# marbl/Mash

Hardware: AMD Instinct MI355X
Metric: pairwise Mash distances/sec (s=1000) (higher is better)
Workload: dtype u64; 1 GPU; mash triangle all-vs-all, 100000 clustered synthetic sketches, k=21 s=1000, 4999950000 pairs/step, per-table job (index build + discover + fill + merge each step), row-block sharded x1; parallelism=rowblock1, rccl_ranks=0

## Files before the change

mash_amd/csrc/host_index.cpp:

```cpp
#include "host_internal.h"
#include "index_build.h"
#ifdef IX_PHASE_CLOCKS
namespace mg { void index_dump_clocks(); }
#endif
#include "sort_bits.h"

namespace {

const uint64_t kTilesLongestRun = 6144;
static const uint64_t kSplitMinRun = 128;

uint64_t longest_label_run(const uint32_t *lab_sorted, uint64_t n)
{
    if (!lab_sorted || n == 0) return 0;
    uint64_t run = 1, longest = 1;
    for (uint64_t a = 1; a < n; a++) {
        run = lab_sorted[a] == lab_sorted[a - 1] ? run + 1 : 1;
        longest = std::max(longest, run);
    }
    return longest;
}

struct SparseIndexBuild {
    mg_ctx *ctx;
    const mg_table *t;
    const uint32_t s;
    const bool clustered;
    const uint32_t split;
    mg_table::Sparse *sp;
    const uint64_t n;
    const std::chrono::steady_clock::time_point t_begin = std::chrono::steady_clock::now();
    bool stop = false;

    bool need_classes = false, dedup = true, want_dense = true, try_cluster = false, try_links = false;
    DevBuf<uint8_t> dc_cls, d_link;
    DevBuf<unsigned long long> dc_last, d_dig, d_dig_sorted, k_a, k_b;
    DevBuf<uint32_t> d_cnt, d_rows_sorted, d_flags, d_nflag, r_a, r_b, l_a, l_b, d_inv, d_lab;
    DevBuf<unsigned char> d_tmp_dup, d_tmp_cl;
    std::vector<uint8_t> hc_cls, link;
    std::vector<uint64_t> hc_last;
    std::vector<uint32_t> hc_nh, inv_v, lab_v;
    const uint32_t *inv = nullptr, *lab_sorted = nullptr;
    uint32_t nflag = 0;
    size_t tb_dup = 0, tb_cl = 0;
    bool cluster_q = false, links_q = false;

    const char *ix_mode = nullptr;
    bool ix_verify = false, ix_tiles = true;
    std::vector<uint32_t> cnt_true, cnt_perm;
    uint32_t max_cnt = 0;
    uint64_t maxv = 0, E_all = 0;
    double dens[65] = {0};
    double dens0 = 0;
    std::vector<uint32_t> rep;
    const uint64_t *H = nullptr;
    mg::IxPlan early_plan;
    DevBuf<unsigned char> d_lb;
    bool lb_made = false;
    bool cnt_stale = false;

    std::vector<uint32_t> cls_of, cls_off, cls_rows, cls_first;

    uint32_t E = 0, end_bit = 0, sort_begin_bit = 0;
    std::vector<mg::DenseGroup> cand_groups;
    std::vector<uint32_t> grp_of_h;
    DevBuf<mg::DenseGroup> d_groups;
    DevBuf<uint32_t> d_grp_of, d_lead_rows, d_val, d_valj, d_cnt_sub, d_off_sub, d_nlead;
    DevBuf<unsigned long long> d_key, d_keyj;
    uint32_t lead_lists = 0, lead_tot[2] = {0, 0}, lead_cap = 0;
    bool lead_ready = false, lead_done = false, cand_prepared = false;
    mg::IxPlan plan;
    size_t temp_bytes = 0;
    DevBuf<unsigned char> temp;
    DevBuf<uint32_t> gs_of;
    DevBuf<unsigned long long> key64_a, key64_b;
    struct Stat { unsigned long long shared; uint32_t max_group, groups, bad, tie_overflow; uint32_t ixf[4]; } h_stat = {0, 0, 0, 0, 0, {0, 0, 0, 0}};
    DevBuf<Stat> d_stat;
    DevBuf<unsigned char> d_slots;
    bool want_order = true, ok = false;
    size_t nshort = 0;
    std::vector<uint32_t> short_cnt;
    hipError_t e = hipSuccess;

    bool built = false;

    SparseIndexBuild(mg_ctx *c, const mg_table *tab, uint32_t sketch_size, bool clustered_variant, mg_table::Sparse *index, uint32_t split_row)
        : ctx(c), t(tab), s(sketch_size), clustered(clustered_variant), split(split_row), sp(index), n(tab->n), dc_cls(c), d_link(c), dc_last(c), d_dig(c),
          d_dig_sorted(c), k_a(c), k_b(c), d_cnt(c), d_rows_sorted(c), d_flags(c), d_nflag(c), r_a(c), r_b(c), l_a(c), l_b(c), d_inv(c),
          d_lab(c), d_tmp_dup(c), d_tmp_cl(c), d_lb(c), d_groups(c), d_grp_of(c), d_lead_rows(c), d_val(c), d_valj(c), d_cnt_sub(c),
          d_off_sub(c), d_nlead(c), d_key(c), d_keyj(c), temp(c), gs_of(c), key64_a(c), key64_b(c), d_stat(c), d_slots(c)
    {
    }

    int unusable(const char *why)
    {
        sp->usable = false;
        sp->why = why;
        stop = true;
        return MG_OK;
    }

    hipError_t counts_to_device()
    {
            if (!cnt_stale) return hipSuccess;
            cnt_stale = false;
            return hipMemcpyAsync(d_cnt, cnt_true.data(), n * 4, hipMemcpyHostToDevice, ctx->stream);
    }

    template <class T> bool take(T **p, size_t count)
    {
        void *q = nullptr;
        if (ctx_malloc(ctx, &q, std::max<size_t>(count, 1) * sizeof(T)) != hipSuccess) return false;
        *p = static_cast<T *>(q);
        return true;
    }

    void drop()
    {
            for (void **q : {(void **)&sp->off, (void **)&sp->keys_sorted, (void **)&sp->gend, (void **)&sp->sorted_rows, (void **)&sp->code_img,
                             (void **)&sp->pos_img, (void **)&sp->short_rows, (void **)&sp->short_cnt, (void **)&sp->counters, (void **)&sp->order,
                             (void **)&sp->rep, (void **)&sp->cls_of, (void **)&sp->cls_off, (void **)&sp->cls_rows, (void **)&sp->cls_first})
                if (*q) { ctx_free(ctx, *q); *q = nullptr; }
    }

    int scan_rows();
    int order_rows();
    int find_copies();
    int lay_out();
    void prepare_candidates();
    void finish_build();
    int build_by_tiles();
    int build_by_sort();
    int check_build();
    int dense_groups();
    int run();
};

int SparseIndexBuild::scan_rows()
{
    need_classes = t->cls.size() != n;
    dedup = !ctx_opt(ctx, "MASHGPU_SPARSE_NO_DEDUP");
    want_dense = true;
    if (const char *v = ctx_opt(ctx, "MASHGPU_COMPARE_DENSE")) want_dense = atoi(v) != 0;
    try_cluster = clustered && n >= 16;
    try_links = !try_cluster && want_dense && n >= 8 && s <= 16384;
    tb_dup = mg::sparse_dup_temp_bytes((uint32_t)n);
    tb_cl = mg::dense_cluster_temp_bytes((uint32_t)n);
    if (d_cnt.alloc(n) != hipSuccess || (need_classes && (dc_cls.alloc(n) != hipSuccess || dc_last.alloc(n) != hipSuccess)) ||
        (dedup && (d_dig.alloc(n) != hipSuccess || d_dig_sorted.alloc(n) != hipSuccess || d_rows_sorted.alloc(n) != hipSuccess ||
                   d_flags.alloc(n) != hipSuccess || d_nflag.alloc(1) != hipSuccess || d_tmp_dup.alloc(std::max<size_t>(tb_dup, 16)) != hipSuccess))) {
        (void)hipGetLastError();
        return unusable("no device memory for the index");
    }
    {
        hipError_t e = hipSuccess;
        if (need_classes) {
            hc_cls.resize(n);
            hc_last.resize(n);
            hc_nh.resize(n);
            e = mg::launch_row_classes(t->hashes, t->nhash, n, t->s, dc_cls, dc_last, ctx->stream);
        }
        if (e == hipSuccess) e = mg::launch_sparse_row_counts(t->nhash, (uint32_t)n, (uint32_t)std::min<uint64_t>(t->s, s), d_cnt, ctx->stream);
        if (e == hipSuccess && dedup) {
            e = mg::launch_sparse_row_digest(t->hashes, t->s, d_cnt, (uint32_t)n, d_dig, ctx->stream);
            if (e == hipSuccess)
                e = mg::launch_sparse_dup_suspects(d_dig, d_cnt, (uint32_t)n, d_tmp_dup, tb_dup, d_dig_sorted, d_rows_sorted, d_flags, d_nflag, ctx->stream);
        }
        if (e == hipSuccess && try_cluster) {
            if (k_a.alloc(4 * n) == hipSuccess && k_b.alloc(4 * n) == hipSuccess && r_a.alloc(4 * n) == hipSuccess && r_b.alloc(4 * n) == hipSuccess &&
                l_a.alloc(n) == hipSuccess && l_b.alloc(n) == hipSuccess && d_inv.alloc(n) == hipSuccess && d_lab.alloc(n) == hipSuccess &&
                d_tmp_cl.alloc(std::max<size_t>(tb_cl, 16)) == hipSuccess) {
                e = mg::dense_cluster_rows(t->hashes, t->s, d_cnt, (uint32_t)n, d_tmp_cl, tb_cl, k_a, k_b, r_a, r_b, l_a, l_b, d_inv, d_lab, ctx->stream, split);
                cluster_q = true;
            } else {
                (void)hipGetLastError();
            }
        }
        if (e == hipSuccess && try_links) {
            if (d_link.alloc(n) == hipSuccess) {
                link.resize(n);
                e = mg::launch_dense_neighbors(t->hashes, t->s, d_cnt, (uint32_t)n, d_link, ctx->stream);
                links_q = true;
            } else {
                (void)hipGetLastError();
            }
        }
        const size_t pin_bytes = 8 * n + 4 * n + 4 * n + 4 * n + 8 + n + n + 64;
        unsigned char *pin = static_cast<unsigned char *>(ctx_pinned(ctx, pin_bytes));
        unsigned long long *p_last = pin ? reinterpret_cast<unsigned long long *>(pin) : nullptr;
        uint32_t *p_nh = pin ? reinterpret_cast<uint32_t *>(pin + 8 * n) : nullptr, *p_inv = pin ? p_nh + n : nullptr, *p_lab = pin ? p_inv + n : nullptr;
        uint32_t *p_nflag = pin ? p_lab + n : &nflag;
        uint8_t *p_cls = pin ? pin + 20 * n + 8 : nullptr, *p_link = pin ? p_cls + n : nullptr;
        if (!pin) {
            if (cluster_q) { inv_v.resize(n); lab_v.resize(n); p_inv = inv_v.data(); p_lab = lab_v.data(); }
            p_nh = hc_nh.data(); p_cls = hc_cls.data(); p_last = reinterpret_cast<unsigned long long *>(hc_last.data()); p_link = link.data();
        }
        if (e == hipSuccess && need_classes) {
            e = hipMemcpyAsync(p_nh, t->nhash, n * 4, hipMemcpyDeviceToHost, ctx->stream);
            if (e == hipSuccess) e = hipMemcpyAsync(p_cls, dc_cls, n, hipMemcpyDeviceToHost, ctx->stream);
            if (e == hipSuccess) e = hipMemcpyAsync(p_last, dc_last, n * 8, hipMemcpyDeviceToHost, ctx->stream);
        }
        if (e == hipSuccess && dedup) e = hipMemcpyAsync(p_nflag, d_nflag, 4, hipMemcpyDeviceToHost, ctx->stream);
        if (e == hipSuccess && cluster_q) {
            e = hipMemcpyAsync(p_inv, d_inv, n * 4, hipMemcpyDeviceToHost, ctx->stream);
            if (e == hipSuccess) e = hipMemcpyAsync(p_lab, d_lab, n * 4, hipMemcpyDeviceToHost, ctx->stream);
        }
        if (e == hipSuccess && links_q) e = hipMemcpyAsync(p_link, d_link, n, hipMemcpyDeviceToHost, ctx->stream);
        const hipError_t es = hipStreamSynchronize(ctx->stream);
        if (e == hipSuccess) e = es;
        if (e == hipSuccess && pin) {
            if (need_classes) {
                memcpy(hc_nh.data(), p_nh, n * 4);
                memcpy(hc_cls.data(), p_cls, n);
                memcpy(hc_last.data(), p_last, n * 8);
            }
            if (dedup) nflag = *p_nflag;
            if (links_q) memcpy(link.data(), p_link, n);
        }
        if (cluster_q) { inv = p_inv; lab_sorted = p_lab; }
        if (e != hipSuccess) return fail(ctx, MG_ERR_HIP, std::string("compare (index: rows, copies, order): ") + hipGetErrorString(e));
    }
    if (need_classes) {
        t->cls.swap(hc_cls);
        t->last.swap(hc_last);
        t->nh.swap(hc_nh);
    }
    if (!links_q) link.clear();
    return MG_OK;
}

int SparseIndexBuild::order_rows()
{
    ix_mode = ctx_opt(ctx, "MASHGPU_SPARSE_INDEX");
    ix_verify = ix_mode && strcmp(ix_mode, "verify") == 0;
    ix_tiles = !ix_mode || strcmp(ix_mode, "sort") != 0;
    cnt_true.assign(n, 0);
    for (uint64_t i = 0; i < n; i++) {
        const uint32_t c = (uint32_t)std::min<uint64_t>(std::min<uint64_t>(t->nh[i], t->s), s);
        cnt_true[i] = c;
        E_all += c;
        max_cnt = std::max(max_cnt, c);
        if (c) {
            const uint64_t last = t->last[i];
            if (last == MG_HASH_PAD) return unusable("a hash equals the padding value");
            maxv = std::max(maxv, last);
            const double d = (double)c / ((double)last + 1.0);
            dens[64 - __builtin_clzll(last | 1ull)] += d;
            dens0 += d;
        }
    }
    H = t->hashes;
    bool keep_table_order = false;
    if (cluster_q && split != 0 && lab_sorted && !ctx_opt(ctx, "MASHGPU_SPLIT_ALWAYS") && longest_label_run(lab_sorted, n) * (uint64_t)s < kSplitMinRun * 1000ull) {
        keep_table_order = true;
        lab_sorted = nullptr;
    }
    if (cluster_q) {
        bool identity = true;
        for (uint64_t a = 0; a < n && identity; a++) identity = inv[a] == a;
        if (!identity && !keep_table_order) {
            void *pi = nullptr, *ph = nullptr;
            if (ctx_malloc(ctx, &pi, n * 4) != hipSuccess || ctx_malloc(ctx, &ph, std::max<uint64_t>(n * t->s, 1) * 8) != hipSuccess) {
                (void)hipGetLastError();
                ctx_free(ctx, pi);
                lab_sorted = nullptr;
            } else {
                sp->inv = static_cast<uint32_t *>(pi);
                sp->phashes = static_cast<uint64_t *>(ph);
                HIP_TRY(ctx, hipMemcpyAsync(sp->inv, d_inv, n * 4, hipMemcpyDeviceToDevice, ctx->stream));
                if (ix_tiles && !(dedup && nflag) && E_all > 0 && E_all < (1ull << 31) && longest_label_run(lab_sorted, n) <= kTilesLongestRun) {
                    early_plan = mg::index_plan((uint32_t)n, (uint32_t)E_all, s, sp->rs, t->s, maxv, dens0, ix_verify);
                    if (early_plan.ok && d_lb.alloc(early_plan.lb_bytes) == hipSuccess) {
                        HIP_TRY(ctx, mg::index_gather_rows(early_plan, t->hashes, sp->inv, d_cnt, sp->phashes, d_lb, ctx->stream));
                        lb_made = true;
                    } else {
                        (void)hipGetLastError();
                    }
                }
                if (!lb_made) HIP_TRY(ctx, mg::launch_dense_gather_rows(t->hashes, t->s, sp->inv, (uint32_t)n, sp->phashes, ctx->stream));
                H = sp->phashes;
                cnt_perm.resize(n);
                for (uint64_t a = 0; a < n; a++) cnt_perm[a] = cnt_true[inv[a]];
                cnt_true.swap(cnt_perm);
                cnt_stale = true;
            }
        }
    } else {
        lab_sorted = nullptr;
    }
    if (want_dense && n >= 8 && s <= 16384 && lab_sorted) {
        link.assign(n, 0);
        for (uint64_t a = 1; a < n; a++) link[a] = (a != split && lab_sorted[a] == lab_sorted[a - 1] && cnt_true[a] && cnt_true[a - 1]) ? 1 : 0;
    } else if (cluster_q && want_dense && n >= 8 && s <= 16384 && d_link.alloc(n) == hipSuccess) {
        link.resize(n);
        HIP_TRY(ctx, counts_to_device());
        HIP_TRY(ctx, mg::launch_dense_neighbors(H, t->s, d_cnt, (uint32_t)n, d_link, ctx->stream));
        HIP_TRY(ctx, hipMemcpyAsync(link.data(), d_link, n, hipMemcpyDeviceToHost, ctx->stream));
        HIP_TRY(ctx, hipStreamSynchronize(ctx->stream));
    } else if (!links_q) {
        (void)hipGetLastError();
        link.clear();
    }
    return MG_OK;
}

int SparseIndexBuild::find_copies()
{
    if (dedup && nflag) {
        HIP_TRY(ctx, counts_to_device());
        HIP_TRY(ctx, mg::launch_sparse_row_digest(H, t->s, d_cnt, (uint32_t)n, d_dig, ctx->stream));
        HIP_TRY(ctx, mg::launch_sparse_dup_suspects(d_dig, d_cnt, (uint32_t)n, d_tmp_dup, tb_dup, d_dig_sorted, d_rows_sorted, d_flags, d_nflag, ctx->stream));
        HIP_TRY(ctx, hipMemcpyAsync(&nflag, d_nflag, 4, hipMemcpyDeviceToHost, ctx->stream));
        HIP_TRY(ctx, hipStreamSynchronize(ctx->stream));
        if (nflag) {
            std::vector<uint32_t> rows_sorted(n), flags(n);
            HIP_TRY(ctx, hipMemcpyAsync(rows_sorted.data(), d_rows_sorted, n * 4, hipMemcpyDeviceToHost, ctx->stream));
            HIP_TRY(ctx, hipMemcpyAsync(flags.data(), d_flags, n * 4, hipMemcpyDeviceToHost, ctx->stream));
            HIP_TRY(ctx, hipStreamSynchronize(ctx->stream));
            std::vector<uint2> pairs;
            pairs.reserve(nflag);
            for (uint64_t k = 1, g0 = 0; k < n; k++) {
                if (flags[k]) pairs.push_back(make_uint2(rows_sorted[k], rows_sorted[g0]));
                else g0 = k;
            }
            DevBuf<uint2> d_pairs(ctx);
            DevBuf<uint32_t> d_eq(ctx);
            if (d_pairs.alloc(pairs.size()) != hipSuccess || d_eq.alloc(pairs.size()) != hipSuccess) { (void)hipGetLastError(); return unusable("no device memory for the index"); }
            std::vector<uint32_t> eq(pairs.size());
            HIP_TRY(ctx, hipMemcpyAsync(d_pairs, pairs.data(), pairs.size() * sizeof(uint2), hipMemcpyHostToDevice, ctx->stream));
            HIP_TRY(ctx, mg::launch_sparse_row_equal(H, t->s, d_cnt, d_pairs, (uint32_t)pairs.size(), d_eq, ctx->stream));
            HIP_TRY(ctx, hipMemcpyAsync(eq.data(), d_eq, pairs.size() * 4, hipMemcpyDeviceToHost, ctx->stream));
            HIP_TRY(ctx, hipStreamSynchronize(ctx->stream));
            for (size_t k = 0; k < pairs.size(); k++)
                if (eq[k]) {
                    if (rep.empty()) { rep.resize(n); for (uint64_t i = 0; i < n; i++) rep[i] = (uint32_t)i; }
                    rep[pairs[k].x] = pairs[k].y;
                    sp->copies++;
                }
        }
    }
    if (sp->copies) {
        cls_of.assign(n, 0xFFFFFFFFu);
        std::vector<uint32_t> size(n, 0);
        for (uint64_t i = 0; i < n; i++) size[rep[i]]++;
        uint32_t ncls = 0, tot = 0;
        for (uint64_t i = 0; i < n; i++)
            if (size[i] >= 2) { cls_of[i] = ncls++; cls_off.push_back(tot); tot += size[i]; }
        cls_off.push_back(tot);
        cls_rows.resize(tot);
        std::vector<uint32_t> fillp(cls_off.begin(), cls_off.end() - 1);
        for (uint64_t i = 0; i < n; i++) {
            const uint32_t k = cls_of[rep[i]];
            if (k != 0xFFFFFFFFu) cls_rows[fillp[k]++] = (uint32_t)i;
        }
        cls_first.resize(tot);
        for (uint32_t k = 0; k < ncls; k++) {
            const uint64_t m = cls_off[k + 1] - cls_off[k];
            sp->cls_pairs += m * (m - 1) / 2;
            for (uint32_t u = cls_off[k]; u < cls_off[k + 1]; u++) cls_first[u] = cls_off[k];
        }
        sp->cls_members = tot;
        if (ncls == 1 && tot == n && cnt_true[0] > 0) sp->one_class = (uint32_t)cnt_true[0];
        if (sp->one_class && ctx->aside_all_copies) ctx->aside_all_copies(sp->one_class);
    }
    return MG_OK;
}

int SparseIndexBuild::lay_out()
{
    uint64_t E64 = 0;
    sp->off_host.resize(n + 1);
    for (uint64_t i = 0; i < n; i++) {
        sp->off_host[i] = (uint32_t)E64;
        const uint64_t c = cnt_true[i];
        if (rep.empty() || rep[i] == i) E64 += c;
        if (E64 >= (1ull << 31)) return unusable("2^31 entries or more");
        if (c < s) sp->short_rows_host.push_back((uint32_t)i);
        if (c == 0) sp->has_empty = true;
    }
    sp->off_host[n] = (uint32_t)E64;
    if (E64 == 0) return unusable("no hashes");
    E = (uint32_t)E64;
    sp->E = E;
    end_bit = (uint32_t)(64 - __builtin_clzll(maxv | 1ull));
    sort_begin_bit = mg::sparse_sort_begin_bit(E, end_bit, ctx_opt(ctx, "MASHGPU_SPARSE_SORT_BITS"), ctx_opt(ctx, "MASHGPU_SPARSE_SORT_ALL_BITS") != nullptr);
    if (sort_begin_bit > 0 && !ctx_opt(ctx, "MASHGPU_SPARSE_SORT_BITS")) sort_begin_bit = mg::sort_begin_bit_from_density(dens, end_bit, sort_begin_bit);
    lead_lists = mg::dense_sublists();
    lead_cap = std::max<uint32_t>(E / 4u / lead_lists + 64u, 256u);
    if (const char *ev = ctx_opt(ctx, "MASHGPU_DENSE_LEAD_CAP")) lead_cap = std::max<uint32_t>((uint32_t)atoi(ev), 1u);
    const bool tiles_hopeless = ix_tiles && !ix_verify && lab_sorted && !ctx_opt(ctx, "MASHGPU_SPARSE_INDEX") &&
                                longest_label_run(lab_sorted, n) > kTilesLongestRun;
    if (ix_tiles && !tiles_hopeless) plan = mg::index_plan((uint32_t)n, E, s, sp->rs, t->s, maxv, dens0, ix_verify);
    else if (tiles_hopeless) plan.why = "a clade of more rows than a bucket's sort takes";
    if (lb_made && !(plan.ok && memcmp(&plan.g, &early_plan.g, sizeof plan.g) == 0)) lb_made = false;
    temp_bytes = std::max(std::max(mg::sparse_order_temp_bytes((uint32_t)n), mg::sparse_order_slice_temp_bytes((uint32_t)n)),
                          mg::sparse_offsets_temp_bytes((uint32_t)n));
    want_order = !ctx_opt(ctx, "MASHGPU_SPARSE_NO_ORDER");
    ok = temp.alloc(std::max<size_t>(temp_bytes, 16)) == hipSuccess && gs_of.alloc(E) == hipSuccess && d_stat.alloc(1) == hipSuccess &&
              d_slots.alloc(std::max(mg::sparse_stat_scratch_bytes(), mg::index_stat_scratch_bytes())) == hipSuccess &&
              (!want_order || (key64_a.alloc(n) == hipSuccess && key64_b.alloc(n) == hipSuccess));
    ok = ok && take(&sp->off, n + 1) && take(&sp->keys_sorted, E) && take(&sp->gend, E) && take(&sp->sorted_rows, E) &&
         take(&sp->code_img, (size_t)n * sp->rs + 64) && take(&sp->pos_img, (size_t)n * sp->rs) && take(&sp->counters, 4) &&
         (!want_order || take(&sp->order, n));
    nshort = sp->short_rows_host.size();
    short_cnt.assign(nshort, 0);
    for (size_t k = 0; k < nshort; k++) short_cnt[k] = cnt_true[sp->short_rows_host[k]];
    if (ok && nshort) ok = take(&sp->short_rows, nshort) && take(&sp->short_cnt, nshort);
    if (ok && sp->copies)
        ok = take(&sp->rep, n) && take(&sp->cls_of, n) && take(&sp->cls_off, cls_off.size()) && take(&sp->cls_rows, cls_rows.size()) &&
             take(&sp->cls_first, cls_first.size());
    e = hipSuccess;
    if (ok && sp->copies) {
        e = hipMemcpyAsync(sp->rep, rep.data(), n * 4, hipMemcpyHostToDevice, ctx->stream);
        if (e == hipSuccess) e = hipMemcpyAsync(sp->cls_of, cls_of.data(), n * 4, hipMemcpyHostToDevice, ctx->stream);
        if (e == hipSuccess) e = hipMemcpyAsync(sp->cls_off, cls_off.data(), cls_off.size() * 4, hipMemcpyHostToDevice, ctx->stream);
        if (e == hipSuccess) e = hipMemcpyAsync(sp->cls_rows, cls_rows.data(), cls_rows.size() * 4, hipMemcpyHostToDevice, ctx->stream);
        if (e == hipSuccess) e = hipMemcpyAsync(sp->cls_first, cls_first.data(), cls_first.size() * 4, hipMemcpyHostToDevice, ctx->stream);
    }
    if (ok && e == hipSuccess) {
        if (rep.empty()) e = mg::launch_sparse_offsets(d_cnt, cnt_stale ? sp->inv : nullptr, (uint32_t)n, temp, sp->off, ctx->stream);
        else e = hipMemcpyAsync(sp->off, sp->off_host.data(), (n + 1) * 4, hipMemcpyHostToDevice, ctx->stream);
        if (e == hipSuccess && nshort) e = hipMemcpyAsync(sp->short_rows, sp->short_rows_host.data(), nshort * 4, hipMemcpyHostToDevice, ctx->stream);
        if (e == hipSuccess && nshort) e = hipMemcpyAsync(sp->short_cnt, short_cnt.data(), nshort * 4, hipMemcpyHostToDevice, ctx->stream);
    }
    return MG_OK;
}

void SparseIndexBuild::prepare_candidates()
{
    if (cand_prepared) return;
    cand_prepared = true;
    if (link.empty() || sp->copies != 0) return;
    for (uint64_t i = 1; i < n;) {
        if (!link[i]) { i++; continue; }
        uint64_t j = i;
        while (j < n && link[j]) j++;
        if (j - (i - 1) >= 8) {
            mg::DenseGroup g{};
            g.g0 = (uint32_t)(i - 1); g.g1 = (uint32_t)j;
            cand_groups.push_back(g);
        }
        i = j + 1;
    }
    if (cand_groups.empty()) return;
    const uint32_t ng = (uint32_t)cand_groups.size();
    grp_of_h.assign(n, 0xFFFFFFFFu);
    for (uint32_t g = 0; g < ng; g++)
        for (uint32_t r = cand_groups[g].g0; r < cand_groups[g].g1; r++) grp_of_h[r] = g;
    const uint64_t room = (uint64_t)lead_lists * lead_cap;
    if (d_groups.alloc(ng) == hipSuccess && d_grp_of.alloc(n) == hipSuccess && d_lead_rows.alloc(4 * n) == hipSuccess && d_nlead.alloc(2) == hipSuccess && d_cnt_sub.alloc(lead_lists) == hipSuccess &&
        d_off_sub.alloc(lead_lists) == hipSuccess && d_key.alloc(room) == hipSuccess && d_val.alloc(room) == hipSuccess && d_keyj.alloc(room) == hipSuccess &&
        d_valj.alloc(room) == hipSuccess &&
        hipMemcpyAsync(d_groups, cand_groups.data(), ng * sizeof(mg::DenseGroup), hipMemcpyHostToDevice, ctx->stream) == hipSuccess &&
        mg::launch_dense_group_rows(d_groups, ng, (uint32_t)n, d_grp_of, d_lead_rows, ctx->stream) == hipSuccess &&
        hipMemsetAsync(d_cnt_sub, 0, lead_lists * 4, ctx->stream) == hipSuccess && hipMemsetAsync(d_nlead, 0, 8, ctx->stream) == hipSuccess) {
        lead_ready = true;
    } else {
        (void)hipGetLastError();
        cand_groups.clear();
    }
}

void SparseIndexBuild::finish_build()
{
    if (e == hipSuccess && want_order)
        e = mg::launch_sparse_row_order(sp->off, sp->code_img, sp->gend, sp->rep, (uint32_t)n, sp->rs, temp, temp_bytes, key64_a, key64_b,
                                        sp->order, ctx->stream);
    if (e == hipSuccess) e = hipMemcpyAsync(&h_stat, d_stat, sizeof(Stat), hipMemcpyDeviceToHost, ctx->stream);
    if (e == hipSuccess) e = hipStreamSynchronize(ctx->stream);
}

int SparseIndexBuild::build_by_tiles()
{
    if (ok && e == hipSuccess && plan.ok) {
        DevBuf<unsigned char> d_tcnt(ctx), d_start(ctx), d_big(ctx), d_pk(ctx), d_tc(ctx);
        if ((lb_made || d_lb.alloc(plan.lb_bytes) == hipSuccess) && d_tcnt.alloc(plan.cnt_bytes) == hipSuccess && d_start.alloc(plan.start_bytes) == hipSuccess &&
            d_big.alloc(plan.big_bytes) == hipSuccess && d_pk.alloc(plan.pk_bytes) == hipSuccess && d_tc.alloc(plan.tc_bytes) == hipSuccess) {
            e = hipMemsetAsync(d_stat, 0, sizeof(Stat), ctx->stream);
            if (e == hipSuccess)
                e = mg::index_build(plan, H, sp->off, d_lb, d_tcnt, d_start, d_big, d_pk, d_tc, sp->keys_sorted, sp->sorted_rows, sp->gend, gs_of, sp->code_img,
                                    sp->pos_img, d_slots, &d_stat.p->shared, &d_stat.p->max_group, &d_stat.p->groups, d_stat.p->ixf, nullptr, ctx->stream,
                                    lb_made ? 1 | 8 : 1);
            DevBuf<uint32_t> d_swapped(ctx);
            if (e == hipSuccess && ctx_opt(ctx, "MASHGPU_IX_DEBUG_SWAP") && d_swapped.alloc(1) == hipSuccess) {
                e = hipMemsetAsync(d_swapped, 0, 4, ctx->stream);
                if (e == hipSuccess) e = mg::index_debug_swap(plan, d_pk, d_start, d_swapped, ctx->stream);
            }
            prepare_candidates();
            mg::IxLeaders lead;
            if (lead_ready) {
                lead.grp_of = d_lead_rows;
                lead.key = d_key;
                lead.val = d_val;
                lead.cnt = d_cnt_sub;
                lead.cap_sub = lead_cap;
                lead.nsub = lead_lists;
            }
            if (e == hipSuccess && ctx->aside_at_sort) ctx->aside_at_sort();
            if (e == hipSuccess)
                e = mg::index_build(plan, H, sp->off, d_lb, d_tcnt, d_start, d_big, d_pk, d_tc, sp->keys_sorted, sp->sorted_rows, sp->gend, gs_of, sp->code_img,
                                    sp->pos_img, d_slots, &d_stat.p->shared, &d_stat.p->max_group, &d_stat.p->groups, d_stat.p->ixf,
                                    lead_ready ? &lead : nullptr, ctx->stream, 2);
            if (e == hipSuccess && lead_ready) {
                e = mg::dense_join_leaders(d_key, d_val, lead_cap, d_keyj, d_valj, d_cnt_sub, d_off_sub, d_nlead, ctx->stream);
                if (e == hipSuccess) e = hipMemcpyAsync(lead_tot, d_nlead, 8, hipMemcpyDeviceToHost, ctx->stream);
            }
            hipEvent_t ev_stats = nullptr;
            if (e == hipSuccess) e = hipMemcpyAsync(&h_stat, d_stat, sizeof(Stat), hipMemcpyDeviceToHost, ctx->stream);
            if (e == hipSuccess) e = hipEventCreateWithFlags(&ev_stats, hipEventDisableTiming);
            if (e == hipSuccess) e = hipEventRecord(ev_stats, ctx->stream);
            if (e == hipSuccess)
                e = mg::index_build(plan, H, sp->off, d_lb, d_tcnt, d_start, d_big, d_pk, d_tc, sp->keys_sorted, sp->sorted_rows, sp->gend, gs_of, sp->code_img,
                                    sp->pos_img, d_slots, &d_stat.p->shared, &d_stat.p->max_group, &d_stat.p->groups, d_stat.p->ixf,
                                    lead_ready ? &lead : nullptr, ctx->stream, 4);
            if (e == hipSuccess && want_order)
                e = mg::launch_sparse_row_order(sp->off, sp->code_img, sp->gend, sp->rep, (uint32_t)n, sp->rs, temp, temp_bytes, key64_a, key64_b,
                                                sp->order, ctx->stream);
            if (ev_stats) {
                const hipError_t ew = e == hipSuccess ? hipEventSynchronize(ev_stats) : hipStreamSynchronize(ctx->stream);
                if (e == hipSuccess) e = ew;
                (void)hipEventDestroy(ev_stats);
            } else {
                (void)hipStreamSynchronize(ctx->stream);
            }
            built = e == hipSuccess && !h_stat.ixf[mg::IXF_DEGENERATE];
            if (built && lead_ready && lead_tot[1] > lead_cap && h_stat.ixf[mg::IXF_NBIG] == 0) {
                e = hipStreamSynchronize(ctx->stream);
                const uint32_t want_cap = lead_tot[1];
                for (void **q : {(void **)&d_key.p, (void **)&d_val.p, (void **)&d_keyj.p, (void **)&d_valj.p})
                    if (*q) { ctx_free(ctx, *q); *q = nullptr; }
                const uint64_t room = (uint64_t)lead_lists * want_cap;
                if (e == hipSuccess && d_key.alloc(room) == hipSuccess && d_val.alloc(room) == hipSuccess && d_keyj.alloc(room) == hipSuccess &&
                    d_valj.alloc(room) == hipSuccess) {
                    lead_cap = want_cap;
                    lead.key = d_key;
                    lead.val = d_val;
                    lead.cap_sub = lead_cap;
                    e = hipMemsetAsync(d_cnt_sub, 0, lead_lists * 4, ctx->stream);
                    if (e == hipSuccess) e = hipMemsetAsync(d_nlead, 0, 8, ctx->stream);
                    if (e == hipSuccess) e = hipMemsetAsync(d_stat.p, 0, offsetof(Stat, bad), ctx->stream);
                    if (e == hipSuccess)
                        e = mg::index_build(plan, H, sp->off, d_lb, d_tcnt, d_start, d_big, d_pk, d_tc, sp->keys_sorted, sp->sorted_rows, sp->gend, gs_of,
                                            sp->code_img, sp->pos_img, d_slots, &d_stat.p->shared, &d_stat.p->max_group, &d_stat.p->groups, d_stat.p->ixf, &lead,
                                            ctx->stream, 2);
                    if (e == hipSuccess) e = mg::dense_join_leaders(d_key, d_val, lead_cap, d_keyj, d_valj, d_cnt_sub, d_off_sub, d_nlead, ctx->stream);
                    if (e == hipSuccess) e = hipMemcpyAsync(lead_tot, d_nlead, 8, hipMemcpyDeviceToHost, ctx->stream);
                    if (e == hipSuccess) e = hipMemcpyAsync(&h_stat, d_stat, sizeof(Stat), hipMemcpyDeviceToHost, ctx->stream);
                    if (e == hipSuccess) e = hipStreamSynchronize(ctx->stream);
                    built = e == hipSuccess && !h_stat.ixf[mg::IXF_DEGENERATE];
                    if (ctx_opt(ctx, "MASHGPU_SPARSE_DBG"))
                        fprintf(stderr, "compare dense: a list of leaders asked for %u entries: found again with that room (%u leaders)\n", want_cap, lead_tot[0]);
                } else {
                    (void)hipGetLastError();
                }
            }
            lead_done = built && lead_ready;
            if (ctx_opt(ctx, "MASHGPU_SPARSE_DBG"))
                fprintf(stderr, "compare sparse: index by tiles: shift %u, %u buckets (%u per window, %u windows), fullest %u, %u beyond the LDS (%u values streamed)%s\n",
                        plan.g.shift, plan.g.Bp, plan.g.BW, plan.g.NW, h_stat.ixf[mg::IXF_MAXBUCKET], h_stat.ixf[mg::IXF_NBIG], h_stat.ixf[mg::IXF_NSTREAMED],
                        h_stat.ixf[mg::IXF_DEGENERATE] ? " -- clumped values: sorted instead" : "");
        } else {
            (void)hipGetLastError();
        }
    } else if (ix_tiles && ctx_opt(ctx, "MASHGPU_SPARSE_DBG")) {
        fprintf(stderr, "compare sparse: index by tiles refused: %s\n", plan.why);
    }
    sp->by_tiles = built;
    prepare_candidates();
#ifdef IX_PHASE_CLOCKS
    if (built && ctx_opt(ctx, "MASHGPU_IX_CLOCKS")) mg::index_dump_clocks();
#endif
    if (ix_verify && !built && ok && e == hipSuccess && !ctx_opt(ctx, "MASHGPU_SPARSE_INDEX_MAY_REFUSE"))
        return fail(ctx, MG_ERR_INVALID, std::string("index verify: the tile build refused this table (") + (plan.ok ? "bucket flags" : plan.why) + ")");
    return MG_OK;
}

int SparseIndexBuild::build_by_sort()
{
    if (ok && e == hipSuccess && (!built || ix_verify)) {
        const size_t sort_bytes = mg::sparse_sort_temp_bytes(E, end_bit, sort_begin_bit);
        DevBuf<unsigned char> temp_sort(ctx), d_ties(ctx);
        DevBuf<uint64_t> keys_a(ctx), v_keys(ctx);
        DevBuf<uint32_t> idx_a(ctx), idx_sorted(ctx), v_rows(ctx), v_gend(ctx), v_gs(ctx), v_code(ctx), v_pos(ctx);
        DevBuf<unsigned long long> d_diff(ctx);
        bool ok2 = temp_sort.alloc(std::max<size_t>(sort_bytes, 16)) == hipSuccess && keys_a.alloc(E) == hipSuccess && idx_a.alloc(E) == hipSuccess &&
                   idx_sorted.alloc(E) == hipSuccess && d_ties.alloc(mg::sparse_tie_scratch_bytes()) == hipSuccess;
        if (ok2 && built)
            ok2 = v_keys.alloc(E) == hipSuccess && v_rows.alloc(E) == hipSuccess && v_gend.alloc(E) == hipSuccess && v_gs.alloc(E) == hipSuccess &&
                  v_code.alloc((size_t)n * sp->rs + 64) == hipSuccess && v_pos.alloc((size_t)n * sp->rs) == hipSuccess && d_diff.alloc(16) == hipSuccess;
        if (!ok2) {
            (void)hipGetLastError();
            ok = false;
        } else {
            const Stat tiles_stat = h_stat;
            uint64_t *o_keys = built ? v_keys.p : sp->keys_sorted;
            uint32_t *o_rows = built ? v_rows.p : sp->sorted_rows, *o_gend = built ? v_gend.p : sp->gend, *o_gs = built ? v_gs.p : gs_of.p,
                     *o_code = built ? v_code.p : sp->code_img, *o_pos = built ? v_pos.p : sp->pos_img;
            for (uint32_t begin_bit = sort_begin_bit;; begin_bit = 0) {
                if (e == hipSuccess) e = hipMemsetAsync(d_stat, 0, sizeof(Stat), ctx->stream);
                if (e == hipSuccess)
                    e = mg::sparse_build_index(H, t->s, sp->off, (uint32_t)n, E, sp->rs, end_bit, temp_sort, sort_bytes, keys_a, idx_a, o_keys, idx_sorted,
                                               idx_a, o_gs, o_rows, o_gend, o_code, o_pos, d_slots, begin_bit, d_ties, &d_stat.p->shared,
                                               &d_stat.p->max_group, &d_stat.p->groups, &d_stat.p->bad, &d_stat.p->tie_overflow, ctx->stream);
                if (built) {
                    if (e == hipSuccess) e = hipMemcpyAsync(&h_stat, d_stat, sizeof(Stat), hipMemcpyDeviceToHost, ctx->stream);
                    if (e == hipSuccess) e = hipStreamSynchronize(ctx->stream);
                } else {
                    finish_build();
                }
                if (e != hipSuccess || (!h_stat.tie_overflow && !h_stat.bad) || begin_bit == 0) break;
                if (ctx_opt(ctx, "MASHGPU_SPARSE_DBG"))
                    fprintf(stderr, "compare sparse: sort on bits [%u, %u) %s: every bit again\n", begin_bit, end_bit,
                            h_stat.bad ? "left values out of order" : "left ties the repair could not take");
            }
            if (built && e == hipSuccess) {
                unsigned long long diff[16];
                for (int k = 0; k < 8; k++) { diff[2 * k] = 0; diff[2 * k + 1] = ~0ull; }
                e = hipMemcpyAsync(d_diff, diff, sizeof diff, hipMemcpyHostToDevice, ctx->stream);
                const uint64_t img = (uint64_t)n * sp->rs;
                if (e == hipSuccess) e = mg::index_verify_words((const uint32_t *)sp->keys_sorted, (const uint32_t *)v_keys.p, nullptr, 0, 2ull * E, d_diff.p + 0, ctx->stream);
                if (e == hipSuccess) e = mg::index_verify_words(sp->sorted_rows, v_rows, nullptr, 0, E, d_diff.p + 2, ctx->stream);
                if (e == hipSuccess) e = mg::index_verify_words(gs_of, v_gs, nullptr, 0, E, d_diff.p + 4, ctx->stream);
                if (e == hipSuccess) e = mg::index_verify_words(sp->gend, v_gend, v_gs, 1, E, d_diff.p + 6, ctx->stream);
                if (e == hipSuccess) e = mg::index_verify_words(sp->code_img, v_code, nullptr, 0, img, d_diff.p + 8, ctx->stream);
                if (e == hipSuccess) e = mg::index_verify_words(sp->pos_img, v_pos, v_code, 2, img, d_diff.p + 10, ctx->stream);
                if (e == hipSuccess) e = hipMemcpyAsync(diff, d_diff, sizeof diff, hipMemcpyDeviceToHost, ctx->stream);
                if (e == hipSuccess) e = hipStreamSynchronize(ctx->stream);
                if (e == hipSuccess) {
                    static const char *names[6] = {"values (32-bit words)", "rows", "group starts", "group ends", "code image", "position image"};
                    std::string msg;
                    for (int k = 0; k < 6; k++)
                        if (diff[2 * k]) msg += std::string(msg.empty() ? "" : "; ") + names[k] + ": " + std::to_string(diff[2 * k]) + " differ, first at " + std::to_string(diff[2 * k + 1]);
                    if (h_stat.shared != tiles_stat.shared || h_stat.max_group != tiles_stat.max_group || h_stat.groups != tiles_stat.groups)
                        msg += std::string(msg.empty() ? "" : "; ") + "statistics: shared " + std::to_string(tiles_stat.shared) + " / " + std::to_string(h_stat.shared) +
                               ", largest group " + std::to_string(tiles_stat.max_group) + " / " + std::to_string(h_stat.max_group) + ", groups " +
                               std::to_string(tiles_stat.groups) + " / " + std::to_string(h_stat.groups);
                    if (!msg.empty()) {
                        char geom[160];
                        snprintf(geom, sizeof geom, " [n %llu, E %u, shift %u, %u buckets, %u per window, %u windows]", (unsigned long long)n, E, plan.g.shift, plan.g.Bp, plan.g.BW, plan.g.NW);
                        sp->usable = false;
                        return fail(ctx, MG_ERR_INVALID, "index verify: tiles / sort -- " + msg + geom);
                    }
                }
            }
        }
    }
    return MG_OK;
}

int SparseIndexBuild::check_build()
{
    if (!ok) { (void)hipGetLastError(); drop(); return unusable("no device memory for the index"); }
    if (e != hipSuccess) { drop(); return fail(ctx, MG_ERR_HIP, std::string("compare (index build): ") + hipGetErrorString(e)); }
    if (h_stat.bad) { drop(); return unusable("sort order inside a value not by row"); }
    sp->G = h_stat.groups;
    sp->shared = h_stat.shared;
    sp->max_group = h_stat.max_group;
    sp->build_ms = std::chrono::duration<double, std::milli>(std::chrono::steady_clock::now() - t_begin).count();
    sp->usable = true;
    return MG_OK;
}

int SparseIndexBuild::dense_groups()
{
    if (!cand_groups.empty()) {
        auto t_dense = std::chrono::steady_clock::now();
        while (!cand_groups.empty()) {
            const uint32_t ng = (uint32_t)cand_groups.size();
            std::vector<uint32_t> &grp_of = grp_of_h;
            DevBuf<uint32_t> d_us(ctx), d_ue(ctx);
            DevBuf<unsigned long long> d_key2(ctx);
            DevBuf<unsigned char> d_tmp(ctx);
            if (d_us.alloc(ng) != hipSuccess || d_ue.alloc(ng) != hipSuccess) { (void)hipGetLastError(); break; }
            const uint32_t L = lead_lists;
            uint32_t *tot = lead_tot, cap_sub = lead_cap;
            hipError_t e2 = hipSuccess;
            if (!lead_done) {
                if (built || !lead_ready) break;
                for (int attempt = 0; e2 == hipSuccess; attempt++) {
                    if (attempt > 0) {
                        for (void **q : {(void **)&d_key.p, (void **)&d_val.p, (void **)&d_keyj.p, (void **)&d_valj.p})
                            if (*q) { ctx_free(ctx, *q); *q = nullptr; }
                        const uint64_t room = (uint64_t)L * cap_sub;
                        if (d_key.alloc(room) != hipSuccess || d_val.alloc(room) != hipSuccess || d_keyj.alloc(room) != hipSuccess || d_valj.alloc(room) != hipSuccess) {
                            (void)hipGetLastError();
                            e2 = hipErrorOutOfMemory;
                            break;
                        }
                    }
                    e2 = mg::dense_find_leaders(sp->sorted_rows, gs_of, sp->gend, d_grp_of, d_groups, E, d_key, d_val, cap_sub, d_keyj, d_valj, d_cnt_sub, d_off_sub,
                                                d_nlead, ctx->stream);
                    if (e2 == hipSuccess) e2 = hipMemcpyAsync(tot, d_nlead, 8, hipMemcpyDeviceToHost, ctx->stream);
                    if (e2 == hipSuccess) e2 = hipStreamSynchronize(ctx->stream);
                    if (e2 != hipSuccess || tot[1] <= cap_sub || attempt >= 1) break;
                    cap_sub = tot[1];
                }
            } else if (tot[1] > cap_sub && ctx_opt(ctx, "MASHGPU_SPARSE_DBG")) {
                fprintf(stderr, "compare dense: a list of leaders asked for %u entries, room for %u: no dense groups for this table\n", tot[1], cap_sub);
            }
            const uint32_t nlead = tot[0];
            if (e2 != hipSuccess || nlead == 0 || tot[1] > cap_sub) { (void)hipGetLastError(); break; }
            uint32_t gbits = 1;
            while ((1u << gbits) < ng) gbits++;
            std::vector<uint32_t> us(ng, 0), ue(ng, 0);
            void *ul = nullptr, *up = nullptr;
            const size_t tb = mg::dense_universe_temp_bytes(nlead);
            if (d_key2.alloc(nlead) != hipSuccess || d_tmp.alloc(std::max<size_t>(tb, 16)) != hipSuccess ||
                ctx_malloc(ctx, &ul, (size_t)nlead * 4) != hipSuccess || ctx_malloc(ctx, &up, (size_t)nlead * 4) != hipSuccess) {
                (void)hipGetLastError();
                ctx_free(ctx, ul);
                break;
            }
            sp->ulist = static_cast<uint32_t *>(ul);
            sp->upos = static_cast<uint32_t *>(up);
            e2 = hipMemsetAsync(d_us, 0, ng * 4, ctx->stream);
            if (e2 == hipSuccess) e2 = hipMemsetAsync(d_ue, 0, ng * 4, ctx->stream);
            if (e2 == hipSuccess)
                e2 = mg::dense_sort_universes(d_keyj, d_valj, nlead, d_tmp, tb, d_key2, sp->ulist, sp->upos, d_us, d_ue, gbits, ctx->stream);
            if (e2 == hipSuccess) e2 = hipMemcpyAsync(us.data(), d_us, ng * 4, hipMemcpyDeviceToHost, ctx->stream);
            if (e2 == hipSuccess) e2 = hipMemcpyAsync(ue.data(), d_ue, ng * 4, hipMemcpyDeviceToHost, ctx->stream);
            if (e2 == hipSuccess) e2 = hipStreamSynchronize(ctx->stream);
            if (e2 != hipSuccess) { (void)hipGetLastError(); break; }
            const uint32_t kMaxWords = mg::dense_max_words();
            std::fill(grp_of.begin(), grp_of.end(), 0xFFFFFFFFu);
            uint32_t xrows = 0, wmax = 0;
            uint64_t words = 0;
            for (uint32_t g = 0; g < ng; g++) {
                mg::DenseGroup G = cand_groups[g];
                G.u = ue[g] > us[g] ? ue[g] - us[g] : 0u;
                G.ustart = us[g];
                G.W = (G.u >> 6) + 1u;
                if (G.u < 32u || G.W > kMaxWords) continue;
                G.xrow0 = xrows;
                G.data_off = words;
                const uint64_t m = G.g1 - G.g0;
                xrows += (uint32_t)m;
                words += ((m + 127) / 128) * mg::dense_block_words(G.W);
                wmax = std::max(wmax, G.W);
                for (uint32_t r = G.g0; r < G.g1; r++) grp_of[r] = (uint32_t)sp->dgroups_host.size();
                sp->dgroups_host.push_back(G);
            }
            if (sp->dgroups_host.empty()) break;
            sp->dn_wmax = wmax;
            sp->dn_xs = ((s + 7u) & ~7u) + 8u;
            void *p1 = nullptr, *p2 = nullptr, *p3 = nullptr, *p4 = nullptr;
            if (ctx_malloc(ctx, &p1, sp->dgroups_host.size() * sizeof(mg::DenseGroup)) != hipSuccess || ctx_malloc(ctx, &p2, n * 4) != hipSuccess ||
                ctx_malloc(ctx, &p3, words * 8) != hipSuccess || ctx_malloc(ctx, &p4, (size_t)xrows * sp->dn_xs * 2) != hipSuccess) {
                (void)hipGetLastError();
                for (void *q : {p1, p2, p3, p4}) ctx_free(ctx, q);
                sp->dgroups_host.clear();
                break;
            }
            sp->dgroups = static_cast<mg::DenseGroup *>(p1);
            sp->grp_of = static_cast<uint32_t *>(p2);
            sp->gdata = static_cast<unsigned long long *>(p3);
            sp->ext = static_cast<uint16_t *>(p4);
            e2 = hipMemcpyAsync(sp->dgroups, sp->dgroups_host.data(), sp->dgroups_host.size() * sizeof(mg::DenseGroup), hipMemcpyHostToDevice, ctx->stream);
            if (e2 == hipSuccess) e2 = hipMemcpyAsync(sp->grp_of, grp_of.data(), n * 4, hipMemcpyHostToDevice, ctx->stream);
            if (e2 == hipSuccess)
                e2 = mg::launch_dense_encode(sp->off, sp->code_img, sp->pos_img, sp->rs, sp->grp_of, sp->dgroups, sp->ulist, sp->upos, sp->gdata,
                                             sp->ext, sp->dn_xs, (uint32_t)n, wmax, ctx->stream,
                                             ctx_opt(ctx, "MASHGPU_DENSE_UL_LDS") ? atoi(ctx_opt(ctx, "MASHGPU_DENSE_UL_LDS")) : -1);
            sp->grp_of_host.swap(grp_of);
            if (e2 != hipSuccess) {
                drop();
                for (void **q : {(void **)&sp->dgroups, (void **)&sp->grp_of, (void **)&sp->gdata, (void **)&sp->ext, (void **)&sp->ulist,
                                 (void **)&sp->upos})
                    if (*q) { ctx_free(ctx, *q); *q = nullptr; }
                sp->dgroups_host.clear();
                sp->usable = false;
                return fail(ctx, MG_ERR_HIP, std::string("compare (index build, dense groups): ") + hipGetErrorString(e2));
            }
            sp->dn_lists = ctx_opt(ctx, "MASHGPU_DENSE_LISTS") != nullptr;
            break;
        }
        if (sp->dgroups_host.empty() && sp->ulist) { ctx_free(ctx, sp->ulist); ctx_free(ctx, sp->upos); sp->ulist = sp->upos = nullptr; }
        sp->build_ms += std::chrono::duration<double, std::milli>(std::chrono::steady_clock::now() - t_dense).count();
        if (ctx_opt(ctx, "MASHGPU_SPARSE_DBG")) {
            uint64_t rows_in = 0;
            for (auto &G : sp->dgroups_host) rows_in += G.g1 - G.g0;
            fprintf(stderr, "compare dense: %zu chains of related rows, %zu groups kept (%llu rows, widest universe %u words)\n", cand_groups.size(),
                    sp->dgroups_host.size(), (unsigned long long)rows_in, sp->dn_wmax);
        }
    }
    if (ctx_opt(ctx, "MASHGPU_SPARSE_DBG"))
        fprintf(stderr, "compare sparse: index of %llu rows (%llu copies of earlier rows), s %u: %u entries, %u distinct, shared %llu, largest run %u, %.2f ms\n",
                (unsigned long long)n, (unsigned long long)sp->copies, s, E, sp->G, (unsigned long long)sp->shared, sp->max_group, sp->build_ms);
    return MG_OK;
}

int SparseIndexBuild::run()
{
    int rc = MG_OK;
    if ((rc = scan_rows()) != MG_OK || stop) return rc;
    if ((rc = order_rows()) != MG_OK || stop) return rc;
    if ((rc = find_copies()) != MG_OK || stop) return rc;
    if ((rc = lay_out()) != MG_OK || stop) return rc;
    if ((rc = build_by_tiles()) != MG_OK || stop) return rc;
    if ((rc = build_by_sort()) != MG_OK || stop) return rc;
    if ((rc = check_build()) != MG_OK || stop) return rc;
    return dense_groups();
}

}

int table_sparse_index(mg_ctx *ctx, const mg_table *t, uint32_t s, bool clustered, mg_table::Sparse **out, uint32_t split)
{
    if (!clustered) split = 0;
    for (mg_table::Sparse *sp : t->sparse)
        if (sp->s == s && sp->clustered == clustered && sp->split == split) { *out = sp; return MG_OK; }
    mg_table::Sparse *sp = new mg_table::Sparse;
    sp->s = s;
    sp->clustered = clustered;
    sp->split = split;
    t->sparse.push_back(sp);
    *out = sp;
    auto unusable = [&](const char *why) { sp->usable = false; sp->why = why; return MG_OK; };
    const uint64_t n = t->n;
    if (n == 0) return unusable("empty table");
    if (n >= (1ull << 31)) return unusable("too many rows");
    sp->rs = mg::sparse_img_stride(s);
    if (n * sp->rs >= (1ull << 32)) return unusable("image index beyond 32 bits");
    HIP_TRY(ctx, hipSetDevice(ctx->device));
    SparseIndexBuild build(ctx, t, s, clustered, sp, split);
    prof_begin(ctx, ctx->prof_index);
    struct ProfEnd { mg_ctx *c; ~ProfEnd() { prof_end(c, c->prof_index); } } prof_end_guard{ctx};
    return build.run();
}
```

mash_amd/csrc/index_build.h:

```cpp
#pragma once
#include <stdint.h>

namespace mg {

struct IxGeom {
    uint32_t n, nblk, E;
    uint32_t shift;
    uint32_t bw_log, BW;
    uint32_t NW, Bp;
    uint32_t rb;
    uint32_t npass;
    uint32_t wgrp;
    uint32_t nseq;
    uint32_t rs;
    uint32_t want_gs;
    uint64_t stride;
};

struct IxLeaders {
    const uint32_t *grp_of = nullptr;
    unsigned long long *key = nullptr;
    uint32_t *val = nullptr;
    uint32_t *cnt = nullptr;
    uint32_t cap_sub = 0, nsub = 0;
};

struct IxPlan {
    IxGeom g;
    bool ok = false;
    const char *why = "";
    size_t lb_bytes = 0, cnt_bytes = 0, start_bytes = 0, big_bytes = 0, pk_bytes = 0, tc_bytes = 0;
};

enum { IXF_NSTREAMED = 0, IXF_DEGENERATE = 1, IXF_MAXBUCKET = 2, IXF_NBIG = 3 };

IxPlan index_plan(uint32_t n, uint32_t E, uint32_t s, uint32_t rs, uint64_t stride, uint64_t maxv, double dens0, bool want_gs);
size_t index_stat_scratch_bytes();
hipError_t index_debug_swap(const IxPlan &plan, void *pk, const void *start, uint32_t *done, hipStream_t stream);
hipError_t index_build(const IxPlan &plan, const uint64_t *hashes, const uint32_t *off, void *lb, void *cnt, void *start, void *big, void *pk, void *tc,
                       uint64_t *keys_sorted, uint32_t *sorted_rows, uint32_t *gend, uint32_t *gs_of, uint32_t *code_img, uint32_t *pos_img,
                       void *stat_scratch, unsigned long long *incidences, uint32_t *max_group, uint32_t *groups, uint32_t *flags,
                       const IxLeaders *leaders, hipStream_t stream, int stages = 7);
hipError_t index_gather_rows(const IxPlan &plan, const uint64_t *hashes, const uint32_t *inv, const uint32_t *cnt_table, uint64_t *out, void *lb,
                             hipStream_t stream);

hipError_t index_verify_words(const uint32_t *a, const uint32_t *b, const uint32_t *cond, uint32_t mode, uint64_t count, unsigned long long *out2,
                              hipStream_t stream);

}
```

mash_amd/csrc/index_build.hip:

```cpp
#ifdef MG_HIP_EMU
#include "hipemu.h"
#else
#include <hip/hip_runtime.h>
#define MG_DYN_SHARED(T, name)                                   \
    extern __shared__ __align__(16) unsigned char name##_raw[]; \
    T *name = reinterpret_cast<T *>(name##_raw)
#endif
#include <stdint.h>

#include <cstdio>
#include <cstdlib>
#include <cstring>

#include "index_build.h"

#ifdef MG_HIP_EMU
#define IX_IN_LANE_ORDER(stmt)                                   \
    for (uint32_t l_ = 0; l_ < 64u; l_++) {                     \
        if ((threadIdx.x & 63u) == l_) { stmt; }                \
        hipemu::wave_sync();                                     \
    }
#else
#define IX_IN_LANE_ORDER(stmt) { stmt; }
#endif

namespace mg {

#if defined(IX_PHASE_CLOCKS) && !defined(MG_HIP_EMU)
__device__ unsigned long long ix_clk[64];
#define IX_CLK_BEGIN() unsigned long long clk_prev_ = threadIdx.x == 0 ? clock64() : 0ull
#define IX_CLK(i)                                                          \
    if (threadIdx.x == 0) {                                               \
        const unsigned long long t_ = clock64();                          \
        atomicAdd(&ix_clk[i], t_ - clk_prev_);                            \
        clk_prev_ = t_;                                                   \
    }
#else
#define IX_CLK_BEGIN() ((void)0)
#define IX_CLK(i) ((void)0)
#endif

constexpr uint32_t IX_RB = 512;
constexpr uint32_t IX_NT = 512;
constexpr uint32_t IX_M = 7;
constexpr uint32_t IX_PCAP = IX_NT * IX_M;
constexpr uint32_t IX_LPR = 8;
constexpr uint32_t IX_BW_MAX = 512;
constexpr uint32_t IX_CAP = 6144;
constexpr uint32_t IX_NT4 = 512;
constexpr uint32_t IX_SUBBITS = 13;
constexpr uint32_t IX_NSUB = 1u << IX_SUBBITS;
constexpr uint32_t IX_SUBLOW = IX_SUBBITS - 3u;
static_assert(IX_SUBBITS == 13 && IX_NT4 == 512, "the ticket slots hold 3 + 13 bits");
constexpr double IX_TMAX = 2560.0;
constexpr double IX_TILE_TARGET = 3072.0;
constexpr uint32_t IX_STAT_SLOTS = 1024;

struct IxStatSlot { unsigned long long inc; uint32_t max_group, groups; };


__device__ __forceinline__ uint32_t ix_block_scan_sum(uint32_t x, uint32_t *part, uint32_t &total)
{
    const uint32_t lane = threadIdx.x & 63u, wid = threadIdx.x >> 6, nw = blockDim.x >> 6;
    uint32_t incl = x;
#pragma unroll
    for (uint32_t d = 1; d < 64u; d <<= 1) {
        const uint32_t y = __shfl_up(incl, d);
        if (lane >= d) incl += y;
    }
    if (lane == 63u) part[wid] = incl;
    __syncthreads();
    uint32_t base = 0, tot = 0;
    for (uint32_t k = 0; k < nw; k++) {
        const uint32_t p = part[k];
        if (k < wid) base += p;
        tot += p;
    }
    __syncthreads();
    total = tot;
    return base + incl - x;
}

__device__ __forceinline__ uint32_t ix_block_scan_max(uint32_t x, uint32_t *part)
{
    const uint32_t lane = threadIdx.x & 63u, wid = threadIdx.x >> 6;
    uint32_t incl = x;
#pragma unroll
    for (uint32_t d = 1; d < 64u; d <<= 1) {
        const uint32_t y = __shfl_up(incl, d);
        if (lane >= d && y > incl) incl = y;
    }
    if (lane == 63u) part[wid] = incl;
    __syncthreads();
    uint32_t base = 0;
    for (uint32_t k = 0; k < wid; k++) base = part[k] > base ? part[k] : base;
    __syncthreads();
    const uint32_t before = __shfl_up(incl, 1u);
    uint32_t ex = lane > 0 ? before : 0u;
    return ex > base ? ex : base;
}

__device__ __forceinline__ bool ix_tile_id(const IxGeom &g, uint32_t &blk, uint32_t &w)
{
    const uint32_t per = gridDim.x >> 3;
    const uint32_t q = (blockIdx.x & 7u) * per + (blockIdx.x >> 3);
    if (q >= g.nseq) return false;
    const uint32_t gsz = g.nblk * g.wgrp;
    const uint32_t wg = q / gsz, rem = q - wg * gsz;
    blk = rem / g.wgrp;
    w = wg * g.wgrp + (rem - blk * g.wgrp);
    return w < g.NW;
}

__global__ __launch_bounds__(256) void ix_gather_offsets_kernel(IxGeom g, const uint64_t *__restrict__ H, const uint32_t *__restrict__ inv,
                                                                const uint32_t *__restrict__ cnt_table, uint64_t *__restrict__ out,
                                                                uint16_t *__restrict__ lb)
{
    const uint32_t a = blockIdx.x, tid = threadIdx.x;
    const uint32_t r = inv[a];
    const uint32_t cnt = cnt_table[r];
    const uint64_t *src = H + (uint64_t)r * g.stride;
    uint64_t *dst = out + (uint64_t)a * g.stride;
    uint16_t *o = lb + (uint64_t)a * (g.NW + 1u);
    const uint32_t wsh = g.shift + g.bw_log;
    for (uint64_t p = tid; p < g.stride; p += 256u) {
        const uint64_t v = src[p];
        dst[p] = v;
        if (p < cnt) {
            const int w = (int)(uint32_t)(v >> wsh);
            const int wp = p > 0 ? (int)(uint32_t)(src[p - 1] >> wsh) : -1;
            for (int x = wp + 1; x <= w; x++) o[x] = (uint16_t)p;
        }
    }
    const int wl = cnt > 0 ? (int)(uint32_t)(src[cnt - 1] >> wsh) : -1;
    for (uint32_t x = (uint32_t)(wl + 1) + tid; x <= g.NW; x += 256u) o[x] = (uint16_t)cnt;
}

__global__ __launch_bounds__(256) void ix_window_offsets_kernel(IxGeom g, const uint64_t *H, const uint32_t *off, uint16_t *lb)
{
    const uint32_t row = blockIdx.x * 4u + (threadIdx.x >> 6), lane = threadIdx.x & 63u;
    if (row < g.n) {
        const uint32_t cnt = off[row + 1] - off[row];
        const uint64_t *src = H + (uint64_t)row * g.stride;
        uint16_t *out = lb + (uint64_t)row * (g.NW + 1u);
        const uint32_t wsh = g.shift + g.bw_log;
        for (uint32_t p = lane; p < cnt; p += 64u) {
            const int w = (int)(uint32_t)(src[p] >> wsh);
            const int wp = p > 0 ? (int)(uint32_t)(src[p - 1] >> wsh) : -1;
            for (int x = wp + 1; x <= w; x++) out[x] = (uint16_t)p;
        }
        const int wl = cnt > 0 ? (int)(uint32_t)(src[cnt - 1] >> wsh) : -1;
        for (uint32_t x = (uint32_t)(wl + 1) + lane; x <= g.NW; x += 64u) out[x] = (uint16_t)cnt;
    }
}

constexpr uint32_t IX_ROUNDS = IX_RB / (IX_NT / IX_LPR);

__global__ __launch_bounds__(IX_NT) void ix_tile_count_kernel(IxGeom g, const uint64_t *__restrict__ H, const uint16_t *__restrict__ lb,
                                                              uint32_t *__restrict__ cnt)
{
    __shared__ uint32_t s_hist[IX_BW_MAX];
    uint32_t blk = 0, w = 0;
    if (!ix_tile_id(g, blk, w)) return;
    const uint32_t tid = threadIdx.x, sub = tid % IX_LPR;
    const uint32_t row0 = blk * IX_RB, nrows = g.n - row0 < IX_RB ? g.n - row0 : IX_RB;
    if (tid < g.BW) s_hist[tid] = 0;
    uint32_t lo[IX_ROUNDS], hi[IX_ROUNDS];
#pragma unroll
    for (uint32_t it = 0; it < IX_ROUNDS; it++) {
        const uint32_t r = it * (IX_NT / IX_LPR) + tid / IX_LPR;
        const uint16_t *p = lb + (uint64_t)(row0 + (r < nrows ? r : 0u)) * (g.NW + 1u) + w;
        const uint32_t a = p[0], b = p[1];
        lo[it] = a;
        hi[it] = r < nrows ? b : a;
    }
    uint64_t v[IX_ROUNDS];
#pragma unroll
    for (uint32_t it = 0; it < IX_ROUNDS; it++) {
        const uint32_t r = it * (IX_NT / IX_LPR) + tid / IX_LPR;
        const bool in = lo[it] + sub < hi[it];
        v[it] = H[in ? (uint64_t)(row0 + r) * g.stride + lo[it] + sub : (uint64_t)row0 * g.stride];
    }
    __syncthreads();
#pragma unroll
    for (uint32_t it = 0; it < IX_ROUNDS; it++) {
        const uint32_t r = it * (IX_NT / IX_LPR) + tid / IX_LPR;
        if (lo[it] + sub < hi[it]) {
            atomicAdd(&s_hist[(uint32_t)(v[it] >> g.shift) & (g.BW - 1u)], 1u);
            const uint64_t *src = H + (uint64_t)(row0 + r) * g.stride;
            for (uint32_t k = lo[it] + sub + IX_LPR; k < hi[it]; k += IX_LPR) atomicAdd(&s_hist[(uint32_t)(src[k] >> g.shift) & (g.BW - 1u)], 1u);
        }
    }
    __syncthreads();
    if (tid < g.BW) cnt[(uint64_t)blk * g.Bp + (uint64_t)w * g.BW + tid] = s_hist[tid];
}

__global__ __launch_bounds__(256) void ix_col_scan_kernel(IxGeom g, uint32_t *cnt, uint32_t *tot)
{
    const uint32_t b = blockIdx.x * 256u + threadIdx.x;
    if (b < g.Bp) {
        uint32_t run = 0;
        for (uint32_t blk0 = 0; blk0 < g.nblk; blk0 += 16u) {
            uint32_t c[16];
#pragma unroll
            for (uint32_t k = 0; k < 16u; k++) c[k] = blk0 + k < g.nblk ? cnt[(uint64_t)(blk0 + k) * g.Bp + b] : 0u;
#pragma unroll
            for (uint32_t k = 0; k < 16u; k++)
                if (blk0 + k < g.nblk) {
                    cnt[(uint64_t)(blk0 + k) * g.Bp + b] = run;
                    run += c[k];
                }
        }
        tot[b] = run;
    }
}

__global__ __launch_bounds__(1024) void ix_bucket_scan_kernel(IxGeom g, uint32_t *start, uint32_t *flags, uint32_t *biglist)
{
    __shared__ uint32_t s_part[16], s_max[16];
    const uint32_t tid = threadIdx.x;
    uint32_t carry = 0, mx = 0;
    for (uint32_t base = 0; base < g.Bp; base += 4096u) {
        const uint32_t b = base + 4u * tid;
        uint32_t c[4], sum = 0;
#pragma unroll
        for (uint32_t k = 0; k < 4u; k++) {
            c[k] = b + k < g.Bp ? start[b + k] : 0u;
            sum += c[k];
            mx = c[k] > mx ? c[k] : mx;
            if (c[k] > IX_CAP) biglist[atomicAdd(&flags[IXF_NBIG], 1u)] = b + k;
        }
        uint32_t total = 0;
        uint32_t run = carry + ix_block_scan_sum(sum, s_part, total);
#pragma unroll
        for (uint32_t k = 0; k < 4u; k++) {
            if (b + k < g.Bp) start[b + k] = run;
            run += c[k];
        }
        carry += total;
    }
    if (tid == 0) start[g.Bp] = carry;
#pragma unroll
    for (uint32_t d = 32; d > 0; d >>= 1) {
        const uint32_t o = __shfl_xor(mx, d);
        mx = o > mx ? o : mx;
    }
    if ((tid & 63u) == 0) s_max[tid >> 6] = mx;
    __syncthreads();
    if (tid == 0) {
        uint32_t m = 0;
        for (uint32_t k = 0; k < 16u; k++) m = s_max[k] > m ? s_max[k] : m;
        flags[IXF_MAXBUCKET] = m;
    }
}

__device__ __forceinline__ uint32_t *ix_tile_sort(uint32_t *src, uint32_t *dst, uint16_t *cnt, uint32_t *part, uint32_t np, uint32_t npass)
{
    const uint32_t tid = threadIdx.x, i0 = tid * IX_M;
    for (uint32_t pass = 0; pass < npass; pass++) {
        const uint32_t sh = 12u + 4u * pass;
#pragma unroll
        for (uint32_t d = 0; d < 16u; d++) cnt[d * IX_NT + tid] = 0;
        uint32_t e[IX_M];
#pragma unroll
        for (uint32_t k = 0; k < IX_M; k++) {
            e[k] = i0 + k < np ? src[i0 + k] : 0xFFFFFFFFu;
            if (i0 + k < np) cnt[((e[k] >> sh) & 15u) * IX_NT + tid]++;
        }
        __syncthreads();
        uint32_t c16[16], sum = 0;
#pragma unroll
        for (uint32_t x = 0; x < 16u; x++) {
            c16[x] = cnt[16u * tid + x];
            sum += c16[x];
        }
        uint32_t total = 0;
        uint32_t run = ix_block_scan_sum(sum, part, total);
#pragma unroll
        for (uint32_t x = 0; x < 16u; x++) {
            cnt[16u * tid + x] = (uint16_t)run;
            run += c16[x];
        }
        __syncthreads();
#pragma unroll
        for (uint32_t k = 0; k < IX_M; k++)
            if (i0 + k < np) {
                uint16_t *c = &cnt[((e[k] >> sh) & 15u) * IX_NT + tid];
                dst[*c] = e[k];
                *c = (uint16_t)(*c + 1u);
            }
        __syncthreads();
        uint32_t *t = src;
        src = dst;
        dst = t;
    }
    return src;
}

constexpr uint32_t IXL_PACK = 0, IXL_PA = IXL_PACK + IX_PCAP * 8u, IXL_PB = IXL_PA + IX_PCAP * 4u, IXL_CNT = IXL_PB + IX_PCAP * 4u,
                   IXL_ROWPRE = IXL_CNT + 16u * IX_NT * 2u, IXL_LO = IXL_ROWPRE + (IX_RB + 2u) * 4u, IXL_HIST = IXL_LO + IX_RB * 2u,
                   IXL_GBASE = IXL_HIST + (IX_BW_MAX + 2u) * 4u, IXL_PART = IXL_GBASE + IX_BW_MAX * 4u, IXL_BYTES = IXL_PART + 64u;

__global__ __launch_bounds__(IX_NT, 4) void ix_tile_partition_kernel(IxGeom g, const uint64_t *__restrict__ H, const uint16_t *__restrict__ lb,
                                                                  const uint32_t *__restrict__ colpre, const uint32_t *__restrict__ start,
                                                                  const uint32_t *__restrict__ flags, uint64_t *__restrict__ pk,
                                                                  uint32_t *__restrict__ slot_img)
{
    MG_DYN_SHARED(unsigned char, lds);
    uint64_t *s_pack = reinterpret_cast<uint64_t *>(lds + IXL_PACK);
    uint32_t *s_pa = reinterpret_cast<uint32_t *>(lds + IXL_PA), *s_pb = reinterpret_cast<uint32_t *>(lds + IXL_PB);
    uint16_t *s_cnt = reinterpret_cast<uint16_t *>(lds + IXL_CNT);
    uint32_t *s_rowpre = reinterpret_cast<uint32_t *>(lds + IXL_ROWPRE);
    uint16_t *s_lo = reinterpret_cast<uint16_t *>(lds + IXL_LO);
    uint32_t *s_hist = reinterpret_cast<uint32_t *>(lds + IXL_HIST);
    uint32_t *s_gbase = reinterpret_cast<uint32_t *>(lds + IXL_GBASE);
    uint32_t *s_part = reinterpret_cast<uint32_t *>(lds + IXL_PART);
    uint32_t blk = 0, w = 0;
    if (!ix_tile_id(g, blk, w)) return;
    const uint32_t tid = threadIdx.x, sub = tid % IX_LPR;
    IX_CLK_BEGIN();
    const uint32_t row0 = blk * IX_RB, nrows = g.n - row0 < IX_RB ? g.n - row0 : IX_RB;
    uint32_t len = 0, gb = 0;
    if (tid < g.BW) {
        const uint32_t bg = w * g.BW + tid;
        gb = start[bg] + colpre[(uint64_t)blk * g.Bp + bg];
    }
    if (tid < nrows) {
        const uint16_t *p = lb + (uint64_t)(row0 + tid) * (g.NW + 1u) + w;
        const uint32_t lo = p[0];
        len = (uint32_t)p[1] - lo;
        s_lo[tid] = (uint16_t)lo;
    }
    uint32_t total = 0;
    const uint32_t pre = ix_block_scan_sum(len, s_part, total);
    if (total == 0) return;
    s_rowpre[tid] = pre;
    if (tid == IX_NT - 1u) s_rowpre[IX_NT] = total;
    if (tid < g.BW) {
        s_gbase[tid] = gb;
        s_hist[tid] = 0;
    }
    __syncthreads();
    IX_CLK(0);
    const uint64_t lowmask = (1ull << g.shift) - 1ull;
    for (uint32_t i0 = 0; i0 < total; i0 += IX_PCAP) {
        const uint32_t np = total - i0 < IX_PCAP ? total - i0 : IX_PCAP;
        uint32_t at[IX_ROUNDS];
        uint64_t v[IX_ROUNDS];
#pragma unroll
        for (uint32_t it = 0; it < IX_ROUNDS; it++) {
            const uint32_t r = it * (IX_NT / IX_LPR) + tid / IX_LPR, rc = r < nrows ? r : 0u;
            const uint32_t rp = s_rowpre[rc], ln = r < nrows ? s_rowpre[rc + 1u] - rp : 0u;
            const uint32_t i = rp + sub;
            const bool in = sub < ln && i >= i0 && i < i0 + np;
            at[it] = in ? i - i0 : 0xFFFFFFFFu;
            v[it] = H[in ? (uint64_t)(row0 + r) * g.stride + s_lo[rc] + sub : (uint64_t)row0 * g.stride];
        }
#pragma unroll
        for (uint32_t it = 0; it < IX_ROUNDS; it++) {
            const uint32_t r = it * (IX_NT / IX_LPR) + tid / IX_LPR;
            if (at[it] != 0xFFFFFFFFu) {
                const uint32_t bl = (uint32_t)(v[it] >> g.shift) & (g.BW - 1u);
                atomicAdd(&s_hist[bl], 1u);
                s_pack[at[it]] = ((v[it] & lowmask) << g.rb) | (uint64_t)(row0 + r);
                s_pa[at[it]] = (bl << 12) | at[it];
            }
        }
#pragma unroll 1
        for (uint32_t r = tid / IX_LPR; r < nrows; r += IX_NT / IX_LPR) {
            const uint32_t rp = s_rowpre[r], ln = s_rowpre[r + 1u] - rp;
            if (ln <= IX_LPR || rp + ln <= i0 || rp >= i0 + np) continue;
            const uint64_t *src = H + (uint64_t)(row0 + r) * g.stride + s_lo[r];
            for (uint32_t k = sub + IX_LPR; k < ln; k += IX_LPR) {
                const uint32_t i = rp + k;
                if (i < i0 || i >= i0 + np) continue;
                const uint64_t x = src[k];
                const uint32_t bl = (uint32_t)(x >> g.shift) & (g.BW - 1u);
                atomicAdd(&s_hist[bl], 1u);
                s_pack[i - i0] = ((x & lowmask) << g.rb) | (uint64_t)(row0 + r);
                s_pa[i - i0] = (bl << 12) | (i - i0);
            }
        }
        __syncthreads();
        IX_CLK(1);
        uint32_t *srt = ix_tile_sort(s_pa, s_pb, s_cnt, s_part, np, g.npass);
        IX_CLK(2);
        uint32_t *s_slot = srt == s_pa ? s_pb : s_pa;
        {
            const uint32_t c = tid < g.BW ? s_hist[tid] : 0u;
            uint32_t tot = 0;
            const uint32_t ex = ix_block_scan_sum(c, s_part, tot);
            if (tid < g.BW) s_hist[tid] = ex;
            if (tid == 0) s_hist[g.BW] = np;
        }
        __syncthreads();
        IX_CLK(3);
        for (uint32_t j = tid; j < np; j += IX_NT) {
            const uint32_t e = srt[j], b = e >> 12, idx = e & 4095u;
            const uint32_t slot = s_gbase[b] + (j - s_hist[b]);
            pk[slot] = s_pack[idx];
            s_slot[idx] = slot;
        }
        __syncthreads();
        IX_CLK(4);
        {
            uint32_t sl[IX_ROUNDS], lo8[IX_ROUNDS];
#pragma unroll
            for (uint32_t it = 0; it < IX_ROUNDS; it++) {
                const uint32_t r = it * (IX_NT / IX_LPR) + tid / IX_LPR;
                sl[it] = s_slot[at[it] != 0xFFFFFFFFu ? at[it] : 0u];
                lo8[it] = s_lo[r < nrows ? r : 0u];
            }
#pragma unroll
            for (uint32_t it = 0; it < IX_ROUNDS; it++) {
                const uint32_t r = it * (IX_NT / IX_LPR) + tid / IX_LPR;
                if (at[it] != 0xFFFFFFFFu) slot_img[(uint64_t)(row0 + r) * g.rs + lo8[it] + sub] = sl[it];
            }
        }
#pragma unroll 1
        for (uint32_t r = tid / IX_LPR; r < nrows; r += IX_NT / IX_LPR) {
            const uint32_t rp = s_rowpre[r], ln = s_rowpre[r + 1u] - rp;
            if (ln <= IX_LPR || rp + ln <= i0 || rp >= i0 + np) continue;
            const uint64_t at0 = (uint64_t)(row0 + r) * g.rs + s_lo[r];
            for (uint32_t k = sub + IX_LPR; k < ln; k += IX_LPR) {
                const uint32_t i = rp + k;
                if (i >= i0 && i < i0 + np) slot_img[at0 + k] = s_slot[i - i0];
            }
        }
        IX_CLK(5);
        uint32_t add = 0;
        if (tid < g.BW) add = s_hist[tid + 1] - s_hist[tid];
        __syncthreads();
        if (tid < g.BW) {
            s_gbase[tid] += add;
            s_hist[tid] = 0;
        }
        __syncthreads();
    }
}

constexpr uint32_t IX5_CH = 32;
constexpr uint32_t IX5_UNR = 4;

__global__ __launch_bounds__(256) void ix_images_kernel(IxGeom g, const uint32_t *__restrict__ off, const uint32_t *__restrict__ flags,
                                                        const uint2 *__restrict__ tc, uint32_t *__restrict__ code_img, uint32_t *pos_img, uint32_t nchunk)
{
    const uint32_t per = gridDim.x >> 3;
    const uint32_t q = (blockIdx.x & 7u) * per + (blockIdx.x >> 3);
    if (q >= g.nblk * nchunk) return;
    const uint32_t blk = q / nchunk, ch = q - blk * nchunk;
    const uint32_t tid = threadIdx.x, quad = tid & 7u, rsub = tid >> 3;
    const uint32_t p0 = ch * IX5_CH + quad * 4u;
    const uint32_t row0 = blk * IX_RB, nrows = g.n - row0 < IX_RB ? g.n - row0 : IX_RB;
    uint32_t cnt_n[IX5_UNR];
    uint32_t sl_n[IX5_UNR][4];
    auto slots = [&](uint32_t rb) {
#pragma unroll
        for (uint32_t u = 0; u < IX5_UNR; u++) {
            const uint32_t r = rb + 32u * u;
            const uint32_t row = row0 + (r < nrows ? r : 0u);
            const uint32_t c = r < nrows ? off[row + 1u] - off[row] : 0u;
            cnt_n[u] = c;
            const uint32_t *src = pos_img + (uint64_t)row * g.rs + (p0 < c ? p0 : 0u);
            sl_n[u][0] = src[0];
            sl_n[u][1] = src[1];
            sl_n[u][2] = src[2];
            sl_n[u][3] = src[3];
        }
    };
    if (rsub < nrows) slots(rsub);
    for (uint32_t rb = rsub; rb < nrows; rb += 32u * IX5_UNR) {
        uint32_t cnt[IX5_UNR];
        uint32_t sl[IX5_UNR][4];
#pragma unroll
        for (uint32_t u = 0; u < IX5_UNR; u++) {
            cnt[u] = cnt_n[u];
#pragma unroll
            for (uint32_t e = 0; e < 4u; e++) sl[u][e] = sl_n[u][e];
        }
        uint2 cp[IX5_UNR][4];
#pragma unroll
        for (uint32_t u = 0; u < IX5_UNR; u++)
#pragma unroll
            for (uint32_t e = 0; e < 4u; e++) cp[u][e] = tc[p0 + e < cnt[u] ? sl[u][e] : 0u];
        if (rb + 32u * IX5_UNR < nrows) slots(rb + 32u * IX5_UNR);
#pragma unroll
        for (uint32_t u = 0; u < IX5_UNR; u++) {
            const uint32_t r = rb + 32u * u;
            if (r < nrows && p0 < g.rs) {
                const uint64_t at = (uint64_t)(row0 + r) * g.rs + p0;
#pragma unroll
                for (uint32_t e = 0; e < 4u; e++) {
                    code_img[at + e] = p0 + e < cnt[u] ? cp[u][e].x : 0xFFFFFFFFu;
                    if (p0 + e < cnt[u]) pos_img[at + e] = cp[u][e].y;
                }
            }
        }
    }
}

__device__ __forceinline__ uint32_t ix_subshift(const IxGeom &g) { return g.shift >= IX_SUBBITS ? g.shift + g.rb - IX_SUBBITS : g.rb; }

constexpr uint32_t IX4_PK = 0, IX4_JX = IX4_PK + IX_CAP * 8u, IX4_H = IX4_JX + IX_CAP * 2u, IX4_MIX = IX4_H + IX_NSUB * 2u,
                   IX4_PART = IX4_MIX + IX_NSUB / 8u, IX4_BYTES = IX4_PART + 64u;

template <bool PART> struct IxBodyPtr { using In = const uint64_t *__restrict__; using Keys = uint64_t *__restrict__; using Rows = uint32_t *__restrict__; };
template <> struct IxBodyPtr<true> { using In = const uint64_t *; using Keys = uint64_t *; using Rows = uint32_t *; };

template <uint32_t PER, bool PART>
__device__ __forceinline__ bool ix_bucket_sort_body(const IxGeom &g, typename IxBodyPtr<PART>::In src, const uint32_t *arr, uint32_t tcbase, uint32_t subshift,
                                                    typename IxBodyPtr<PART>::Keys keys_sorted, typename IxBodyPtr<PART>::Rows sorted_rows, uint32_t *__restrict__ gend,
                                                    uint32_t *__restrict__ gs_of, uint2 *__restrict__ tc, IxStatSlot *stat, uint32_t *flags,
                                                    const IxLeaders &lead, uint64_t *s_pk, uint16_t *s_jx, uint32_t *s_h, uint32_t *s_mixed,
                                                    uint32_t *s_part, uint32_t b, uint32_t G0, uint32_t N)
{
    const uint32_t tid = threadIdx.x, lane = tid & 63u, wave = tid >> 6;
    IX_CLK_BEGIN();
    for (uint32_t x = tid; x < IX_NSUB / 2u; x += IX_NT4) s_h[x] = 0;
    if (tid < IX_NSUB / 32u) s_mixed[tid] = 0;
    uint64_t v[PER];
    uint32_t sa[PER];
    uint32_t am[PART ? PER : 1u];
#pragma unroll
    for (uint32_t k = 0; k < PER; k++) {
        const uint32_t j = tid + k * IX_NT4;
        const bool in = j < N;
        const uint64_t x = src[in ? j : 0u];
        v[k] = x;
        if constexpr (PART) am[k] = arr[in ? j : 0u];
        const uint32_t sub0 = (uint32_t)(x >> subshift) & (IX_NSUB - 1u);
        if (in) s_jx[j] = (uint16_t)(((sub0 >> IX_SUBLOW) << 13) | (sub0 & ((1u << IX_SUBLOW) - 1u)));
    }
    __syncthreads();
    IX_CLK(32);
    uint16_t *s_tk = s_jx;
    for (uint32_t j0 = 0; j0 < N; j0 += 256u) {
        uint32_t tag[4];
#pragma unroll
        for (uint32_t u = 0; u < 4u; u++) {
            const uint32_t j = j0 + 64u * u + lane;
            tag[u] = j < N ? (uint32_t)s_tk[j] : 0xFFFFu;
        }
        uint32_t old[4];
#pragma unroll
        for (uint32_t u = 0; u < 4u; u++) {
            const uint32_t j = j0 + 64u * u + lane;
            const bool mine = (tag[u] >> 13) == wave && j < N;
            const uint32_t sub = (wave << IX_SUBLOW) | (tag[u] & ((1u << IX_SUBLOW) - 1u));
            const uint32_t h16 = (sub & 1u) * 16u;
            uint32_t o = 0;
            IX_IN_LANE_ORDER(if (mine) o = atomicAdd(&s_h[sub >> 1], 1u << h16));
            old[u] = (o >> h16) & 0xFFFFu;
        }
#pragma unroll
        for (uint32_t u = 0; u < 4u; u++) {
            const uint32_t j = j0 + 64u * u + lane;
            if ((tag[u] >> 13) == wave && j < N) s_tk[j] = (uint16_t)((wave << 13) | old[u]);
        }
    }
    __syncthreads();
    IX_CLK(33);
    {
        uint32_t wv[8], sum = 0;
#pragma unroll
        for (uint32_t x = 0; x < 8u; x++) {
            wv[x] = s_h[8u * tid + x];
            sum += (wv[x] & 0xFFFFu) + (wv[x] >> 16);
        }
        uint32_t total = 0;
        uint32_t run = ix_block_scan_sum(sum, s_part, total);
#pragma unroll
        for (uint32_t x = 0; x < 8u; x++) {
            const uint32_t lo = wv[x] & 0xFFFFu, hi = wv[x] >> 16;
            s_h[8u * tid + x] = run | ((run + lo) << 16);
            run += lo + hi;
        }
    }
    const uint16_t *cs = reinterpret_cast<const uint16_t *>(s_h);
#pragma unroll
    for (uint32_t k = 0; k < PER; k++) {
        const uint32_t j = tid + k * IX_NT4;
        sa[k] = (uint32_t)s_tk[j < N ? j : 0u] & 0x1FFFu;
    }
    __syncthreads();
    IX_CLK(34);
#pragma unroll
    for (uint32_t k = 0; k < PER; k++) {
        const uint32_t j = tid + k * IX_NT4;
        if (j < N) {
            const uint32_t sub = (uint32_t)(v[k] >> subshift) & (IX_NSUB - 1u);
            const uint32_t q = (uint32_t)cs[sub] + sa[k];
            s_pk[q] = v[k];
            s_jx[q] = (uint16_t)j;
        }
    }
    __syncthreads();
    IX_CLK(35);
    {
        uint32_t diff = 0;
#pragma unroll
        for (uint32_t k = 0; k < PER; k++) {
            const uint32_t q = tid + k * IX_NT4;
            const uint64_t me = s_pk[q < N ? q : 0u];
            const uint32_t sub = (uint32_t)(me >> subshift) & (IX_NSUB - 1u);
            if (q < N && (s_pk[cs[sub]] >> g.rb) != (me >> g.rb)) diff |= 1u << k;
        }
        if (diff) {
#pragma unroll
            for (uint32_t k = 0; k < PER; k++)
                if ((diff >> k) & 1u) {
                    const uint32_t sub = (uint32_t)(s_pk[tid + k * IX_NT4] >> subshift) & (IX_NSUB - 1u);
                    atomicOr(&s_mixed[sub >> 5], 1u << (sub & 31u));
                }
        }
    }
    __syncthreads();
#pragma unroll
    for (uint32_t k = 0; k < PER; k++) {
        const uint32_t q = tid + k * IX_NT4;
        const bool in = q < N;
        const uint32_t qc = in ? q : 0u;
        const uint64_t me = s_pk[qc];
        const uint32_t jv = s_jx[qc];
        const uint32_t sub = (uint32_t)(me >> subshift) & (IX_NSUB - 1u);
        uint32_t nq = qc;
        if (in && ((s_mixed[sub >> 5] >> (sub & 31u)) & 1u)) {
            const uint32_t a = cs[sub], e = sub + 1u < IX_NSUB ? (uint32_t)cs[sub + 1u] : N;
            {
                uint32_t r = 0;
                if (subshift - g.rb <= 32u) {
                    const uint32_t low = (uint32_t)(me >> g.rb);
                    for (uint32_t x = a; x < e; x++) {
                        const uint32_t lx = (uint32_t)(s_pk[x] >> g.rb);
                        r += (lx < low || (lx == low && x < qc)) ? 1u : 0u;
                    }
                } else {
                    const uint64_t low = me >> g.rb;
                    for (uint32_t x = a; x < e; x++) {
                        const uint64_t lx = s_pk[x] >> g.rb;
                        r += (lx < low || (lx == low && x < qc)) ? 1u : 0u;
                    }
                }
                nq = a + r;
            }
        }
        v[k] = me;
        sa[k] = nq | (jv << 16);
    }
    __syncthreads();
#pragma unroll
    for (uint32_t k = 0; k < PER; k++) {
        const uint32_t q = tid + k * IX_NT4;
        if (q < N) {
            s_pk[sa[k] & 0xFFFFu] = v[k];
            s_jx[sa[k] & 0xFFFFu] = (uint16_t)(sa[k] >> 16);
        }
    }
    __syncthreads();
    IX_CLK(36);
    uint16_t *inv = reinterpret_cast<uint16_t *>(s_h);
    unsigned long long *s_hb = reinterpret_cast<unsigned long long *>(s_mixed);
    int unordered = 0;
#pragma unroll
    for (uint32_t k = 0; k < PER; k++) {
        const uint32_t q = tid + k * IX_NT4;
        const bool in = q < N;
        const uint32_t qc = in ? q : 0u;
        const uint64_t w = s_pk[qc], prev = s_pk[qc > 0 ? qc - 1u : 0u];
        const bool head = in && (q == 0 || (w >> g.rb) != (prev >> g.rb));
        if (in && q > 0 && w <= prev) unordered = 1;
        if (in) inv[s_jx[q]] = (uint16_t)q;
        const unsigned long long bal = __ballot(head);
        if (lane == 0 && q < N) s_hb[q >> 6] = bal;
    }
    unordered = __syncthreads_or(unordered);
    if (unordered) {
        if (tid == 0) flags[IXF_DEGENERATE] = 1u;
        return false;
    }
    IX_CLK(37);
    auto group_start = [&](uint32_t q) -> uint32_t {
        uint32_t w = q >> 6;
        unsigned long long m = s_hb[w] & (~0ull >> (63u - (q & 63u)));
        while (m == 0) m = s_hb[--w];
        return (w << 6) + 63u - (uint32_t)__builtin_clzll(m);
    };
    auto is_head = [&](uint32_t q) -> bool { return (s_hb[q >> 6] >> (q & 63u)) & 1ull; };
    const uint64_t rowmask = (1ull << g.rb) - 1ull;
    const uint64_t vbase = (uint64_t)b << g.shift;
    unsigned long long inc = 0;
    uint32_t heads = 0, glen = 0, lmask = 0;
    uint32_t gsr[PER], grpr[PER], g0r[PER], g1r[PER];
#pragma unroll
    for (uint32_t k = 0; k < PER; k++) {
        const uint32_t q = tid + k * IX_NT4;
        const bool in = q < N;
        const uint32_t qc = in ? q : 0u;
        const uint32_t gs = group_start(qc);
        const bool last = qc + 1u == N || is_head(qc + 1u);
        gsr[k] = gs;
        const bool look = lead.grp_of != nullptr && in && !(last && qc == gs);
        const uint32_t *gp = lead.grp_of + 4ull * (uint32_t)(s_pk[qc] & rowmask);
        grpr[k] = look ? gp[0] : 0xFFFFFFFFu;
        g0r[k] = look ? gp[1] : 0u;
        g1r[k] = look ? gp[2] : 0u;
        inc += in ? q - gs : 0u;
        heads += (in && q == gs) ? 1u : 0u;
        const uint32_t len = (in && last) ? q + 1u - gs : 0u;
        glen = len > glen ? len : glen;
    }
#pragma unroll
    for (uint32_t k = 0; k < PER; k++) {
        const uint32_t q = tid + k * IX_NT4;
        if (q < N) {
            const uint64_t w = s_pk[q];
            const uint32_t gs = gsr[k];
            const bool last = q + 1u == N || is_head(q + 1u);
            keys_sorted[G0 + q] = vbase | (w >> g.rb);
            sorted_rows[G0 + q] = (uint32_t)(w & rowmask);
            if (gs_of) gs_of[G0 + q] = G0 + gs;
            if (last) gend[G0 + gs] = G0 + q + 1u;
            if (grpr[k] != 0xFFFFFFFFu) {
                const bool first = q == gs || (uint32_t)(s_pk[q - 1u] & rowmask) < g0r[k];
                const bool more = !last && (uint32_t)(s_pk[q + 1u] & rowmask) < g1r[k];
                if (first && more) lmask |= 1u << k;
            }
        }
    }
    IX_CLK(38);
#pragma unroll
    for (uint32_t d = 32; d > 0; d >>= 1) {
        inc += __shfl_xor(inc, d);
        heads += __shfl_xor(heads, d);
        const uint32_t o = __shfl_xor(glen, d);
        glen = o > glen ? o : glen;
    }
    __shared__ unsigned long long s_inc[IX_NT4 / 64];
    __shared__ uint32_t s_len[IX_NT4 / 64], s_heads[IX_NT4 / 64];
    if (lane == 0) {
        s_inc[wave] = inc;
        s_len[wave] = glen;
        s_heads[wave] = heads;
    }
    uint32_t ltotal = 0, lbase = 0;
    if (lead.grp_of) lbase = ix_block_scan_sum((uint32_t)__popc(lmask), s_part, ltotal);
    else __syncthreads();
    if (tid == 0) {
        if (ltotal) s_part[15] = atomicAdd(&lead.cnt[b & (lead.nsub - 1u)], ltotal);
        unsigned long long t = 0;
        uint32_t m = 0, h = 0;
        for (uint32_t k = 0; k < IX_NT4 / 64u; k++) {
            t += s_inc[k];
            m = s_len[k] > m ? s_len[k] : m;
            h += s_heads[k];
        }
        IxStatSlot *sl = stat + (b & (IX_STAT_SLOTS - 1u));
        if (t) atomicAdd(&sl->inc, t);
        if (m > 1u) atomicMax(&sl->max_group, m);
        atomicAdd(&sl->groups, h);
    }
    IX_CLK(39);
#pragma unroll
    for (uint32_t k = 0; k < PER; k++) {
        const uint32_t j = tid + k * IX_NT4;
        if (j < N) {
            const uint32_t q = inv[j], gs = group_start(q);
            const bool last = q + 1u == N || is_head(q + 1u);
            const uint32_t shared = (gs == q && last) ? 0u : 1u;
            uint32_t at = j;
            if constexpr (PART) at = am[k];
            tc[tcbase + at] = make_uint2(((G0 + gs) << 1) | shared, G0 + q);
        }
    }
    IX_CLK(40);
    if (ltotal) {
        __syncthreads();
        const uint32_t sub = b & (lead.nsub - 1u);
        uint32_t at = s_part[15] + lbase;
#pragma unroll
        for (uint32_t k = 0; k < PER; k++) {
            if ((lmask >> k) & 1u) {
                const uint32_t q = tid + k * IX_NT4;
                if (at < lead.cap_sub) {
                    const uint64_t slot = (uint64_t)sub * lead.cap_sub + at;
                    lead.key[slot] = ((unsigned long long)grpr[k] << 32) | (unsigned long long)(G0 + gsr[k]);
                    lead.val[slot] = G0 + q;
                }
                at++;
            }
        }
    }
    IX_CLK(41);
    return true;
}

__global__ __launch_bounds__(IX_NT4, 4) void ix_bucket_sort_kernel(IxGeom g, const uint64_t *pk, const uint32_t *start, uint64_t *keys_sorted,
                                                                uint32_t *sorted_rows, uint32_t *gend, uint32_t *gs_of, uint2 *tc,
                                                                IxStatSlot *stat, uint32_t *flags, IxLeaders lead)
{
    MG_DYN_SHARED(unsigned char, lds);
    uint64_t *s_pk = reinterpret_cast<uint64_t *>(lds + IX4_PK);
    uint16_t *s_jx = reinterpret_cast<uint16_t *>(lds + IX4_JX);
    uint32_t *s_h = reinterpret_cast<uint32_t *>(lds + IX4_H);
    uint32_t *s_mixed = reinterpret_cast<uint32_t *>(lds + IX4_MIX);
    uint32_t *s_part = reinterpret_cast<uint32_t *>(lds + IX4_PART);
    const uint32_t b = blockIdx.x;
    const uint32_t G0 = start[b], N = start[b + 1] - G0;
    if (N == 0 || N > IX_CAP) return;
    const uint32_t per = (N + IX_NT4 - 1u) / IX_NT4;
    const uint32_t subshift = ix_subshift(g);
#define IX_BODY(P)                                                                                                                          \
    (void)ix_bucket_sort_body<P, false>(g, pk + G0, nullptr, G0, subshift, keys_sorted, sorted_rows, gend, gs_of, tc, stat, flags, lead, s_pk, s_jx, \
                                        s_h, s_mixed, s_part, b, G0, N)
    if (per <= 3u) IX_BODY(3);
    else if (per <= 4u) IX_BODY(4);
    else if (per <= 5u) IX_BODY(5);
    else if (per <= 6u) IX_BODY(6);
    else if (per <= 8u) IX_BODY(8);
    else IX_BODY(12);
#undef IX_BODY
}

constexpr uint32_t IXB_CS1 = IX4_BYTES, IXB_CS2 = IXB_CS1 + IX_NSUB * 4u, IXB_BYTES = IXB_CS2 + IX_NSUB * 4u;
constexpr uint32_t IXB_CH = 4096;
constexpr uint32_t IXB_W = 0, IXB_ARR = IXB_W + IXB_CH * 8u, IXB_TAG = IXB_ARR + IXB_CH * 4u;
static_assert(IXB_TAG + IXB_CH * 2u <= IX4_H, "the staging area lies in the body's entry arrays");

struct IxOut {
    uint64_t *keys_sorted;
    uint32_t *sorted_rows, *gend, *gs_of;
    uint2 *tc;
    IxStatSlot *stat;
    uint32_t *flags;
};

__device__ __forceinline__ uint32_t ix_big_first(const uint32_t *cs, uint32_t k) { return k ? cs[k - 1u] : 0u; }

__device__ __forceinline__ void ix_big_split(const uint64_t *src_w, const uint32_t *src_arr, uint64_t *dst_w, uint32_t *dst_arr, uint32_t count,
                                             uint32_t sshift, uint32_t *cs, unsigned char *lds, uint32_t *s_part)
{
    uint64_t *s_w = reinterpret_cast<uint64_t *>(lds + IXB_W);
    uint32_t *s_arr = reinterpret_cast<uint32_t *>(lds + IXB_ARR);
    uint16_t *s_tag = reinterpret_cast<uint16_t *>(lds + IXB_TAG);
    const uint32_t tid = threadIdx.x, lane = tid & 63u, wave = tid >> 6;
    for (uint32_t x = tid; x < IX_NSUB; x += IX_NT4) cs[x] = 0;
    __syncthreads();
    for (uint32_t j = tid; j < count; j += IX_NT4) atomicAdd(&cs[(uint32_t)(src_w[j] >> sshift) & (IX_NSUB - 1u)], 1u);
    __syncthreads();
    {
        constexpr uint32_t W = IX_NSUB / IX_NT4;
        uint32_t c[W], sum = 0;
#pragma unroll
        for (uint32_t x = 0; x < W; x++) {
            c[x] = cs[W * tid + x];
            sum += c[x];
        }
        uint32_t total = 0;
        uint32_t run = ix_block_scan_sum(sum, s_part, total);
#pragma unroll
        for (uint32_t x = 0; x < W; x++) {
            cs[W * tid + x] = run;
            run += c[x];
        }
    }
    for (uint32_t j0 = 0; j0 < count; j0 += IXB_CH) {
        __syncthreads();
        for (uint32_t x = tid; x < IXB_CH; x += IX_NT4) {
            const uint32_t j = j0 + x, jc = j < count ? j : 0u;
            const uint64_t w = src_w[jc];
            const uint32_t sub0 = (uint32_t)(w >> sshift) & (IX_NSUB - 1u);
            s_w[x] = w;
            s_arr[x] = src_arr ? src_arr[jc] : j;
            s_tag[x] = (uint16_t)(((sub0 >> IX_SUBLOW) << 13) | (sub0 & ((1u << IX_SUBLOW) - 1u)));
        }
        __syncthreads();
        const uint32_t xe = count - j0 < IXB_CH ? count - j0 : IXB_CH;
        for (uint32_t x0 = 0; x0 < xe; x0 += 256u) {
            uint32_t tag[4];
#pragma unroll
            for (uint32_t u = 0; u < 4u; u++) tag[u] = s_tag[x0 + 64u * u + lane];
#pragma unroll
            for (uint32_t u = 0; u < 4u; u++) {
                const uint32_t x = x0 + 64u * u + lane;
                const bool mine = (tag[u] >> 13) == wave && x < xe;
                const uint32_t sub = (wave << IX_SUBLOW) | (tag[u] & ((1u << IX_SUBLOW) - 1u));
                uint32_t at = 0;
                IX_IN_LANE_ORDER(if (mine) at = atomicAdd(&cs[sub], 1u));
                if (mine) {
                    dst_w[at] = s_w[x];
                    dst_arr[at] = s_arr[x];
                }
            }
        }
    }
    __threadfence();
    __syncthreads();
}

__device__ __forceinline__ bool ix_big_one_value(const IxGeom &g, const uint64_t *src_w, uint32_t m)
{
    const uint64_t low0 = src_w[0] >> g.rb;
    int bad = 0;
    for (uint32_t q = threadIdx.x; q < m; q += IX_NT4) bad |= (src_w[q] >> g.rb) != low0 ? 1 : 0;
    return __syncthreads_or(bad) == 0;
}

__device__ __forceinline__ bool ix_big_value(const IxGeom &g, const uint64_t *src_w, const uint32_t *src_arr, const IxOut &o, const IxLeaders &lead,
                                             uint32_t *s_row, uint32_t *s_part, uint32_t b, uint32_t tcbase, uint32_t gs, uint32_t m)
{
    const uint32_t tid = threadIdx.x;
    const uint64_t rowmask = (1ull << g.rb) - 1ull;
    const uint64_t vbase = (uint64_t)b << g.shift;
    int bad = 0;
    for (uint32_t q0 = 0; q0 < m; q0 += IX_NT4) {
        const uint32_t q = q0 + tid;
        const bool in = q < m, more_after = q + 1u < m;
        const uint64_t w = src_w[in ? q : 0u];
        const uint32_t ar = src_arr[in ? q : 0u];
        const uint32_t next_row = (uint32_t)(src_w[more_after ? q + 1u : 0u] & rowmask);
        const uint32_t row = (uint32_t)(w & rowmask);
        s_row[tid + 1u] = row;
        __syncthreads();
        const uint32_t prev_row = s_row[tid];
        if (in && q > 0 && prev_row >= row) bad = 1;
        bool isl = false;
        uint32_t grp = 0xFFFFFFFFu;
        if (lead.grp_of != nullptr && in) {
            const uint32_t *gp = lead.grp_of + 4ull * row;
            grp = gp[0];
            const bool first = q == 0 || prev_row < gp[1];
            isl = grp != 0xFFFFFFFFu && first && more_after && next_row < gp[2];
        }
        __syncthreads();
        if (tid == IX_NT4 - 1u) s_row[0] = row;
        if (in) {
            o.keys_sorted[gs + q] = vbase | (w >> g.rb);
            o.sorted_rows[gs + q] = row;
            if (o.gs_of) o.gs_of[gs + q] = gs;
            o.tc[tcbase + ar] = make_uint2((gs << 1) | 1u, gs + q);
        }
        if (lead.grp_of != nullptr) {
            uint32_t ltotal = 0;
            const uint32_t lbase = ix_block_scan_sum(isl ? 1u : 0u, s_part, ltotal);
            if (ltotal) {
                const uint32_t sub = b & (lead.nsub - 1u);
                if (tid == 0) s_part[15] = atomicAdd(&lead.cnt[sub], ltotal);
                __syncthreads();
                const uint32_t at = s_part[15] + lbase;
                if (isl && at < lead.cap_sub) {
                    const uint64_t slot = (uint64_t)sub * lead.cap_sub + at;
                    lead.key[slot] = ((unsigned long long)grp << 32) | (unsigned long long)gs;
                    lead.val[slot] = gs + q;
                }
                __syncthreads();
            }
        }
    }
    bad = __syncthreads_or(bad);
    if (bad) {
        if (tid == 0) o.flags[IXF_DEGENERATE] = 1u;
        return false;
    }
    if (tid == 0) {
        o.gend[gs] = gs + m;
        atomicAdd(&o.flags[IXF_NSTREAMED], 1u);
        IxStatSlot *sl = o.stat + (b & (IX_STAT_SLOTS - 1u));
        atomicAdd(&sl->inc, (unsigned long long)m * (unsigned long long)(m - 1u) / 2ull);
        atomicMax(&sl->max_group, m);
        atomicAdd(&sl->groups, 1u);
    }
    return true;
}

template <int LEVEL>
__device__ bool ix_big_walk(const IxGeom &g, const uint64_t *src_w, const uint32_t *src_arr, uint64_t *alt_w, uint32_t *alt_arr, uint32_t gpos,
                            uint32_t count, uint32_t sshift, const uint32_t *cs, uint32_t *cs_next, const IxOut &o, const IxLeaders &lead,
                            unsigned char *lds, uint32_t b, uint32_t tcbase)
{
    uint64_t *s_pk = reinterpret_cast<uint64_t *>(lds + IX4_PK);
    uint16_t *s_jx = reinterpret_cast<uint16_t *>(lds + IX4_JX);
    uint32_t *s_h = reinterpret_cast<uint32_t *>(lds + IX4_H);
    uint32_t *s_mixed = reinterpret_cast<uint32_t *>(lds + IX4_MIX);
    uint32_t *s_part = reinterpret_cast<uint32_t *>(lds + IX4_PART);
    const uint32_t sshift_next = sshift - g.rb >= IX_SUBBITS ? sshift - IX_SUBBITS : g.rb;
    uint32_t sub = 0;
    while (sub < IX_NSUB) {
        const uint32_t a = ix_big_first(cs, sub);
        if (a == count) break;
        uint32_t lo = sub, hi = IX_NSUB;
        if (count - a <= IX_CAP) lo = hi;
        while (hi - lo > 1u) {
            const uint32_t mid = (lo + hi) >> 1;
            if (ix_big_first(cs, mid) - a <= IX_CAP) lo = mid;
            else hi = mid;
        }
        bool ok = true;
        if (lo == sub) {
            const uint32_t m = cs[sub] - a;
            if (ix_big_one_value(g, src_w + a, m)) {
                ok = ix_big_value(g, src_w + a, src_arr + a, o, lead, reinterpret_cast<uint32_t *>(lds + IX4_PK), s_part, b, tcbase, gpos + a, m);
            } else if (LEVEL == 1 && sshift > g.rb) {
                if constexpr (LEVEL == 1) {
                    ix_big_split(src_w + a, src_arr + a, alt_w + a, alt_arr + a, m, sshift_next, cs_next, lds, s_part);
                    ok = ix_big_walk<2>(g, alt_w + a, alt_arr + a, nullptr, nullptr, gpos + a, m, sshift_next, cs_next, nullptr, o, lead, lds, b, tcbase);
                }
            } else {
                if (threadIdx.x == 0) o.flags[IXF_DEGENERATE] = 1u;
                ok = false;
            }
            sub++;
        } else {
            const uint32_t cnt = ix_big_first(cs, lo) - a;
            if (cnt)
                ok = ix_bucket_sort_body<IX_CAP / IX_NT4, true>(g, src_w + a, src_arr + a, tcbase, lo == sub + 1u ? sshift_next : sshift, o.keys_sorted,
                                                                o.sorted_rows, o.gend, o.gs_of, o.tc, o.stat, o.flags, lead, s_pk, s_jx, s_h, s_mixed, s_part,
                                                                b, gpos + a, cnt);
            sub = lo;
        }
        if (!ok) return false;
        __syncthreads();
    }
    return true;
}

__global__ __launch_bounds__(IX_NT4, 2) void ix_big_bucket_kernel(IxGeom g, uint64_t *pk, const uint32_t *start, const uint32_t *biglist,
                                                               uint64_t *keys_sorted, uint32_t *sorted_rows, uint32_t *gend, uint32_t *gs_of, uint2 *tc,
                                                               IxStatSlot *stat, uint32_t *flags, IxLeaders lead)
{
    MG_DYN_SHARED(unsigned char, lds);
    uint32_t *s_part = reinterpret_cast<uint32_t *>(lds + IX4_PART);
    uint32_t *cs1 = reinterpret_cast<uint32_t *>(lds + IXB_CS1), *cs2 = reinterpret_cast<uint32_t *>(lds + IXB_CS2);
    const IxOut o{keys_sorted, sorted_rows, gend, gs_of, tc, stat, flags};
    const uint32_t nbig = flags[IXF_NBIG];
    const uint32_t sshift = ix_subshift(g);
    for (uint32_t i = blockIdx.x; i < nbig; i += gridDim.x) {
        const uint32_t b = biglist[i];
        const uint32_t G0 = start[b], N = start[b + 1] - G0;
        ix_big_split(pk + G0, nullptr, keys_sorted + G0, sorted_rows + G0, N, sshift, cs1, lds, s_part);
        if (!ix_big_walk<1>(g, keys_sorted + G0, sorted_rows + G0, pk + G0, gend + G0, G0, N, sshift, cs1, cs2, o, lead, lds, b, G0)) return;
        __syncthreads();
    }
}

__global__ __launch_bounds__(256) void ix_stat_reduce_kernel(const IxStatSlot *stat, unsigned long long *incidences, uint32_t *max_group, uint32_t *groups)
{
    unsigned long long inc = 0;
    uint32_t m = 0, gr = 0;
    for (uint32_t i = threadIdx.x; i < IX_STAT_SLOTS; i += 256u) {
        inc += stat[i].inc;
        m = stat[i].max_group > m ? stat[i].max_group : m;
        gr += stat[i].groups;
    }
    if (inc) atomicAdd(incidences, inc);
    if (m) atomicMax(max_group, m);
    if (gr) atomicAdd(groups, gr);
}

__global__ __launch_bounds__(256) void ix_fill_u32_kernel(uint32_t *p, uint64_t count, uint32_t v)
{
    const uint64_t stride = (uint64_t)gridDim.x * 256u;
    for (uint64_t i = (uint64_t)blockIdx.x * 256u + threadIdx.x; i < count; i += stride) p[i] = v;
}

__global__ __launch_bounds__(256) void ix_verify_kernel(const uint32_t *a, const uint32_t *b, const uint32_t *cond, uint32_t mode, uint64_t count,
                                                        unsigned long long *out)
{
    const uint64_t stride = (uint64_t)gridDim.x * 256u;
    for (uint64_t i = (uint64_t)blockIdx.x * 256u + threadIdx.x; i < count; i += stride) {
        if (mode == 1u && cond[i] != (uint32_t)i) continue;
        if (mode == 2u && cond[i] == 0xFFFFFFFFu) continue;
        if (a[i] != b[i]) {
            atomicAdd(&out[0], 1ull);
            atomicMin(&out[1], (unsigned long long)i);
        }
    }
}

hipError_t index_verify_words(const uint32_t *a, const uint32_t *b, const uint32_t *cond, uint32_t mode, uint64_t count, unsigned long long *out2,
                              hipStream_t stream)
{
    if (count == 0) return hipSuccess;
    uint64_t blocks = (count + 1023u) / 1024u;
    if (blocks > 8192u) blocks = 8192u;
    hipLaunchKernelGGL(ix_verify_kernel, dim3((uint32_t)blocks), dim3(256), 0, stream, a, b, cond, mode, count, out2);
    return hipGetLastError();
}


size_t index_stat_scratch_bytes() { return sizeof(IxStatSlot) * IX_STAT_SLOTS; }

#if defined(IX_PHASE_CLOCKS) && !defined(MG_HIP_EMU)
void index_dump_clocks()
{
    unsigned long long h[64];
    if (hipMemcpyFromSymbol(h, HIP_SYMBOL(ix_clk), sizeof h) != hipSuccess) return;
    static const char *k3[] = {"prologue (lb, scan, gbase)", "loads + pack", "tile sort", "bucket scan", "pk + slots to LDS", "slot image"};
    static const char *k4[] = {"zero + load", "tickets", "counter scan + ticket read", "scatter", "mixed mark + fix-up + write back", "heads + inverse", "out by position + leaders", "statistics + leaders' scan", "tc by arrival", "leaders out"};
    unsigned long long t3 = 0, t4 = 0;
    for (int i = 0; i < 6; i++) t3 += h[i];
    for (int i = 0; i < 10; i++) t4 += h[32 + i];
    for (int i = 0; i < 6; i++) fprintf(stderr, "ix clocks K3 %-34s %6.2f %%\n", k3[i], 100.0 * h[i] / (t3 ? t3 : 1));
    for (int i = 0; i < 10; i++) fprintf(stderr, "ix clocks K4 %-34s %6.2f %%\n", k4[i], 100.0 * h[32 + i] / (t4 ? t4 : 1));
    memset(h, 0, sizeof h);
    (void)hipMemcpyToSymbol(HIP_SYMBOL(ix_clk), h, sizeof h);
}
#endif

IxPlan index_plan(uint32_t n, uint32_t E, uint32_t s, uint32_t rs, uint64_t stride, uint64_t maxv, double dens0, bool want_gs)
{
    IxPlan p;
    IxGeom &g = p.g;
    g = IxGeom{};
    if (n == 0 || E == 0) { p.why = "empty"; return p; }
    if (s > 65535u) { p.why = "sketch size beyond 16-bit positions"; return p; }
    g.n = n;
    g.E = E;
    g.rs = rs;
    g.stride = stride;
    g.want_gs = want_gs ? 1u : 0u;
    g.nblk = (n + IX_RB - 1u) / IX_RB;
    g.rb = 1;
    while (g.rb < 32u && (1ull << g.rb) < (uint64_t)n) g.rb++;
    if (!(dens0 > 0.0)) { p.why = "no density"; return p; }
    uint32_t shift = 0;
    while (shift < 63u && dens0 * (double)(1ull << (shift + 1u)) <= IX_TMAX) shift++;
    if (shift > 64u - g.rb) shift = 64u - g.rb;
    if (shift > 63u) shift = 63u;
    g.shift = shift;
    const uint64_t B = (maxv >> shift) + 1ull;
    if (B > (1ull << 22)) { p.why = "too many buckets (values far from evenly spread)"; return p; }
    uint32_t bw_log = 0;
    while (bw_log < 9u && (1ull << (bw_log + 1u)) <= IX_BW_MAX && shift + bw_log + 1u <= 63u && (1ull << bw_log) < B &&
           (double)E * (double)(2u << bw_log) / ((double)g.nblk * (double)B) <= IX_TILE_TARGET)
        bw_log++;
    g.bw_log = bw_log;
    g.BW = 1u << bw_log;
    g.NW = (uint32_t)((B + g.BW - 1u) / g.BW);
    g.Bp = g.NW * g.BW;
    g.npass = (bw_log + 3u) / 4u;
    g.wgrp = 8;
    const uint64_t nseq = (uint64_t)((g.NW + g.wgrp - 1u) / g.wgrp) * g.wgrp * g.nblk;
    if (nseq >= (1ull << 30)) { p.why = "too many tiles"; return p; }
    g.nseq = (uint32_t)nseq;
    p.lb_bytes = (size_t)n * (g.NW + 1u) * 2u;
    p.cnt_bytes = (size_t)g.nblk * g.Bp * 4u;
    p.start_bytes = ((size_t)g.Bp + 1u) * 4u;
    p.pk_bytes = (size_t)E * 8u;
    p.tc_bytes = (size_t)E * 8u;
    p.big_bytes = ((size_t)E / IX_CAP + 2u) * 4u;
    if (p.lb_bytes > ((size_t)2 << 30) || p.cnt_bytes > ((size_t)2 << 30)) { p.why = "scratch of the tiles too large"; return p; }
    p.ok = true;
    return p;
}

hipError_t index_gather_rows(const IxPlan &plan, const uint64_t *hashes, const uint32_t *inv, const uint32_t *cnt_table, uint64_t *out, void *lb_v,
                             hipStream_t stream)
{
    if (!plan.ok) return hipErrorInvalidValue;
    hipLaunchKernelGGL(ix_gather_offsets_kernel, dim3(plan.g.n), dim3(256), 0, stream, plan.g, hashes, inv, cnt_table, out, static_cast<uint16_t *>(lb_v));
    return hipGetLastError();
}

__global__ __launch_bounds__(64) void ix_debug_swap_kernel(IxGeom g, uint64_t *pk, const uint32_t *start, uint32_t *done)
{
    if (threadIdx.x != 0) return;
    for (uint32_t b = 0; b < g.Bp; b++) {
        const uint32_t a = start[b], e = start[b + 1];
        if (e - a < 2u || e - a > IX_CAP) continue;
        for (uint32_t j = a; j + 1u < e; j++) {
            if ((pk[j] >> g.rb) == (pk[j + 1] >> g.rb)) {
                const uint64_t t = pk[j];
                pk[j] = pk[j + 1];
                pk[j + 1] = t;
                done[0] = 1u;
                return;
            }
        }
    }
}

hipError_t index_debug_swap(const IxPlan &plan, void *pk_v, const void *start_v, uint32_t *done, hipStream_t stream)
{
    if (!plan.ok) return hipErrorInvalidValue;
    hipLaunchKernelGGL(ix_debug_swap_kernel, dim3(1), dim3(64), 0, stream, plan.g, static_cast<uint64_t *>(pk_v), static_cast<const uint32_t *>(start_v), done);
    return hipGetLastError();
}

hipError_t index_build(const IxPlan &plan, const uint64_t *hashes, const uint32_t *off, void *lb_v, void *cnt_v, void *start_v, void *big_v, void *pk_v, void *tc_v,
                       uint64_t *keys_sorted, uint32_t *sorted_rows, uint32_t *gend, uint32_t *gs_of, uint32_t *code_img, uint32_t *pos_img,
                       void *stat_scratch, unsigned long long *incidences, uint32_t *max_group, uint32_t *groups, uint32_t *flags,
                       const IxLeaders *leaders, hipStream_t stream, int stages)
{
    if (!plan.ok) return hipErrorInvalidValue;
    const IxGeom g = plan.g;
    uint16_t *lb = static_cast<uint16_t *>(lb_v);
    uint32_t *cnt = static_cast<uint32_t *>(cnt_v), *start = static_cast<uint32_t *>(start_v);
    uint64_t *pk = static_cast<uint64_t *>(pk_v);
    uint2 *tc = static_cast<uint2 *>(tc_v);
    hipError_t e = hipSuccess;
    if (stages & 1) {
        e = hipFuncSetAttribute(reinterpret_cast<const void *>(ix_tile_partition_kernel), hipFuncAttributeMaxDynamicSharedMemorySize, (int)IXL_BYTES);
        if (e != hipSuccess) return e;
        const uint32_t tiles = 8u * ((g.nseq + 7u) / 8u);
        if (!(stages & 8)) hipLaunchKernelGGL(ix_window_offsets_kernel, dim3((g.n + 3u) / 4u), dim3(256), 0, stream, g, hashes, off, lb);
        hipLaunchKernelGGL(ix_tile_count_kernel, dim3(tiles), dim3(IX_NT), 0, stream, g, hashes, (const uint16_t *)lb, cnt);
        hipLaunchKernelGGL(ix_col_scan_kernel, dim3((g.Bp + 255u) / 256u), dim3(256), 0, stream, g, cnt, start);
        hipLaunchKernelGGL(ix_bucket_scan_kernel, dim3(1), dim3(1024), 0, stream, g, start, flags, static_cast<uint32_t *>(big_v));
        e = hipGetLastError();
        if (e != hipSuccess) return e;
        hipLaunchKernelGGL(ix_tile_partition_kernel, dim3(tiles), dim3(IX_NT), IXL_BYTES, stream, g, hashes, (const uint16_t *)lb, (const uint32_t *)cnt,
                           (const uint32_t *)start, (const uint32_t *)flags, pk, pos_img);
        e = hipGetLastError();
        if (e != hipSuccess) return e;
    }
    if (stages & 2) {
        e = hipFuncSetAttribute(reinterpret_cast<const void *>(ix_bucket_sort_kernel), hipFuncAttributeMaxDynamicSharedMemorySize, (int)IX4_BYTES);
        if (e == hipSuccess) e = hipFuncSetAttribute(reinterpret_cast<const void *>(ix_big_bucket_kernel), hipFuncAttributeMaxDynamicSharedMemorySize, (int)IXB_BYTES);
        if (e != hipSuccess) return e;
        e = hipMemsetAsync(stat_scratch, 0, index_stat_scratch_bytes(), stream);
        if (e != hipSuccess) return e;
        hipLaunchKernelGGL(ix_bucket_sort_kernel, dim3(g.Bp), dim3(IX_NT4), IX4_BYTES, stream, g, (const uint64_t *)pk, (const uint32_t *)start, keys_sorted,
                           sorted_rows, gend, g.want_gs ? gs_of : (uint32_t *)nullptr, tc, static_cast<IxStatSlot *>(stat_scratch), flags,
                           leaders ? *leaders : IxLeaders());
        hipLaunchKernelGGL(ix_big_bucket_kernel, dim3(256), dim3(IX_NT4), IXB_BYTES, stream, g, pk, (const uint32_t *)start,
                           (const uint32_t *)big_v, keys_sorted, sorted_rows, gend, g.want_gs ? gs_of : (uint32_t *)nullptr, tc,
                           static_cast<IxStatSlot *>(stat_scratch), flags, leaders ? *leaders : IxLeaders());
        hipLaunchKernelGGL(ix_stat_reduce_kernel, dim3(1), dim3(256), 0, stream, static_cast<const IxStatSlot *>(stat_scratch), incidences, max_group, groups);
    }
    if (!(stages & 4)) return hipGetLastError();
    {
        const uint32_t nchunk = (g.rs + IX5_CH - 1u) / IX5_CH;
        const uint32_t pieces = 8u * ((g.nblk * nchunk + 7u) / 8u);
        hipLaunchKernelGGL(ix_images_kernel, dim3(pieces), dim3(256), 0, stream, g, off, (const uint32_t *)flags, (const uint2 *)tc, code_img, pos_img, nchunk);
    }
    return hipGetLastError();
}

}
```

Before: 435.1 billion pairs/s.

## Fuse index front pass and read hashes through a row map instead of copying

The clustered index build used to gather a permuted copy of the whole hash table before building the tiles. It now reads the original table indirectly through the row map. A new front kernel computes the window offsets and the per-block bucket counts in one pass when the counters fit in LDS, which drops the separate count kernel. The permuted copy is now made lazily, only for the paths that still need it (the dup digest and the general sort). In exchange, every hash load in the partition pass goes through an extra indirection with less contiguous row access, and a degenerate flag now lets the partition kernels skip their work.

```diff
diff --git a/mash_amd/csrc/host_index.cpp b/mash_amd/csrc/host_index.cpp
--- a/mash_amd/csrc/host_index.cpp
+++ b/mash_amd/csrc/host_index.cpp
@@ -54,9 +54,12 @@
     double dens0 = 0;
     std::vector<uint32_t> rep;
     const uint64_t *H = nullptr;
+    const uint32_t *rowmap = nullptr;
     mg::IxPlan early_plan;
-    DevBuf<unsigned char> d_lb;
-    bool lb_made = false;
+    DevBuf<unsigned char> d_lb, d_tcnt;
+    bool lb_made = false, cnt_made = false;
+    bool stat_zeroed = false;
+    bool ix_front = true;
     bool cnt_stale = false;
 
     std::vector<uint32_t> cls_of, cls_off, cls_rows, cls_first;
@@ -87,7 +90,7 @@
     SparseIndexBuild(mg_ctx *c, const mg_table *tab, uint32_t sketch_size, bool clustered_variant, mg_table::Sparse *index, uint32_t split_row)
         : ctx(c), t(tab), s(sketch_size), clustered(clustered_variant), split(split_row), sp(index), n(tab->n), dc_cls(c), d_link(c), dc_last(c), d_dig(c),
           d_dig_sorted(c), k_a(c), k_b(c), d_cnt(c), d_rows_sorted(c), d_flags(c), d_nflag(c), r_a(c), r_b(c), l_a(c), l_b(c), d_inv(c),
-          d_lab(c), d_tmp_dup(c), d_tmp_cl(c), d_lb(c), d_groups(c), d_grp_of(c), d_lead_rows(c), d_val(c), d_valj(c), d_cnt_sub(c),
+          d_lab(c), d_tmp_dup(c), d_tmp_cl(c), d_lb(c), d_tcnt(c), d_groups(c), d_grp_of(c), d_lead_rows(c), d_val(c), d_valj(c), d_cnt_sub(c),
           d_off_sub(c), d_nlead(c), d_key(c), d_keyj(c), temp(c), gs_of(c), key64_a(c), key64_b(c), d_stat(c), d_slots(c)
     {
     }
@@ -105,6 +108,36 @@
             if (!cnt_stale) return hipSuccess;
             cnt_stale = false;
             return hipMemcpyAsync(d_cnt, cnt_true.data(), n * 4, hipMemcpyHostToDevice, ctx->stream);
+    }
+
+    hipError_t need_copy_with_offsets()
+    {
+        void *ph = sp->phashes;
+        hipError_t ec = ph ? hipSuccess : ctx_malloc(ctx, &ph, std::max<uint64_t>(n * t->s, 1) * 8);
+        if (ec != hipSuccess) return ec;
+        sp->phashes = static_cast<uint64_t *>(ph);
+        ec = mg::index_gather_rows(early_plan, t->hashes, sp->inv, d_cnt, sp->phashes, d_lb, ctx->stream);
+        if (ec != hipSuccess) return ec;
+        H = sp->phashes;
+        rowmap = nullptr;
+        lb_made = true;
+        if (ctx_opt(ctx, "MASHGPU_SPARSE_DBG")) fprintf(stderr, "compare sparse: clustered copy of the table made for the tiles (MASHGPU_IX_FRONT=0)\n");
+        return hipSuccess;
+    }
+
+    hipError_t need_copy(const char *who)
+    {
+        if (H) return hipSuccess;
+        void *ph = sp->phashes;
+        hipError_t ec = ph ? hipSuccess : ctx_malloc(ctx, &ph, std::max<uint64_t>(n * t->s, 1) * 8);
+        if (ec != hipSuccess) return ec;
+        sp->phashes = static_cast<uint64_t *>(ph);
+        ec = mg::launch_dense_gather_rows(t->hashes, t->s, sp->inv, (uint32_t)n, sp->phashes, ctx->stream);
+        if (ec != hipSuccess) return ec;
+        H = sp->phashes;
+        rowmap = nullptr;
+        if (ctx_opt(ctx, "MASHGPU_SPARSE_DBG")) fprintf(stderr, "compare sparse: clustered copy of the table made for %s\n", who);
+        return hipSuccess;
     }
 
     template <class T> bool take(T **p, size_t count)
@@ -234,6 +267,7 @@
     ix_mode = ctx_opt(ctx, "MASHGPU_SPARSE_INDEX");
     ix_verify = ix_mode && strcmp(ix_mode, "verify") == 0;
     ix_tiles = !ix_mode || strcmp(ix_mode, "sort") != 0;
+    if (const char *v = ctx_opt(ctx, "MASHGPU_IX_FRONT")) ix_front = atoi(v) != 0;
     cnt_true.assign(n, 0);
     for (uint64_t i = 0; i < n; i++) {
         const uint32_t c = (uint32_t)std::min<uint64_t>(std::min<uint64_t>(t->nh[i], t->s), s);
@@ -259,30 +293,54 @@
         bool identity = true;
         for (uint64_t a = 0; a < n && identity; a++) identity = inv[a] == a;
         if (!identity && !keep_table_order) {
-            void *pi = nullptr, *ph = nullptr;
-            if (ctx_malloc(ctx, &pi, n * 4) != hipSuccess || ctx_malloc(ctx, &ph, std::max<uint64_t>(n * t->s, 1) * 8) != hipSuccess) {
+            void *pi = nullptr;
+            bool copy_refused = false;
+            if (ctx_malloc(ctx, &pi, n * 4) != hipSuccess) {
                 (void)hipGetLastError();
-                ctx_free(ctx, pi);
                 lab_sorted = nullptr;
             } else {
                 sp->inv = static_cast<uint32_t *>(pi);
-                sp->phashes = static_cast<uint64_t *>(ph);
+                H = nullptr;
+                rowmap = sp->inv;
                 HIP_TRY(ctx, hipMemcpyAsync(sp->inv, d_inv, n * 4, hipMemcpyDeviceToDevice, ctx->stream));
                 if (ix_tiles && !(dedup && nflag) && E_all > 0 && E_all < (1ull << 31) && longest_label_run(lab_sorted, n) <= kTilesLongestRun) {
-                    early_plan = mg::index_plan((uint32_t)n, (uint32_t)E_all, s, sp->rs, t->s, maxv, dens0, ix_verify);
-                    if (early_plan.ok && d_lb.alloc(early_plan.lb_bytes) == hipSuccess) {
-                        HIP_TRY(ctx, mg::index_gather_rows(early_plan, t->hashes, sp->inv, d_cnt, sp->phashes, d_lb, ctx->stream));
-                        lb_made = true;
+                    early_plan = mg::index_plan((uint32_t)n, (uint32_t)E_all, s, sp->rs, t->s, maxv, dens0, ix_verify, ix_front ? ~(size_t)0 : 0);
+                    if (early_plan.ok && ix_front) {
+                        if (d_lb.alloc(early_plan.lb_bytes) == hipSuccess && d_tcnt.alloc(early_plan.cnt_bytes) == hipSuccess && d_stat.alloc(1) == hipSuccess) {
+                            HIP_TRY(ctx, hipMemsetAsync(d_stat, 0, sizeof(Stat), ctx->stream));
+                            stat_zeroed = true;
+                            HIP_TRY(ctx, mg::index_front(early_plan, t->hashes, sp->inv, d_cnt, nullptr, d_lb, d_tcnt, d_stat.p->ixf, ctx->stream));
+                            lb_made = true;
+                            cnt_made = early_plan.front;
+                            if (ctx_opt(ctx, "MASHGPU_SPARSE_DBG"))
+                                fprintf(stderr, "compare sparse: index front through the row map, no clustered copy: %s\n",
+                                        cnt_made ? "window offsets and block counts in one pass" : "window offsets (the blocks' counters do not fit the LDS)");
+                        } else {
+                            (void)hipGetLastError();
+                        }
+                    } else if (early_plan.ok && d_lb.alloc(early_plan.lb_bytes) == hipSuccess) {
+                        if (need_copy_with_offsets() != hipSuccess) {
+                            (void)hipGetLastError();
+                            d_lb.free();
+                            copy_refused = true;
+                        }
                     } else {
                         (void)hipGetLastError();
                     }
                 }
-                if (!lb_made) HIP_TRY(ctx, mg::launch_dense_gather_rows(t->hashes, t->s, sp->inv, (uint32_t)n, sp->phashes, ctx->stream));
-                H = sp->phashes;
-                cnt_perm.resize(n);
-                for (uint64_t a = 0; a < n; a++) cnt_perm[a] = cnt_true[inv[a]];
-                cnt_true.swap(cnt_perm);
-                cnt_stale = true;
+                if (!lb_made && (copy_refused || need_copy("an index that does not go the tiles' early way") != hipSuccess)) {
+                    (void)hipGetLastError();
+                    ctx_free(ctx, sp->inv);
+                    sp->inv = nullptr;
+                    H = t->hashes;
+                    rowmap = nullptr;
+                    lab_sorted = nullptr;
+                } else {
+                    cnt_perm.resize(n);
+                    for (uint64_t a = 0; a < n; a++) cnt_perm[a] = cnt_true[inv[a]];
+                    cnt_true.swap(cnt_perm);
+                    cnt_stale = true;
+                }
             }
         }
     } else {
@@ -307,6 +365,7 @@
 int SparseIndexBuild::find_copies()
 {
     if (dedup && nflag) {
+        HIP_TRY(ctx, need_copy("the copy suspects"));
         HIP_TRY(ctx, counts_to_device());
         HIP_TRY(ctx, mg::launch_sparse_row_digest(H, t->s, d_cnt, (uint32_t)n, d_dig, ctx->stream));
         HIP_TRY(ctx, mg::launch_sparse_dup_suspects(d_dig, d_cnt, (uint32_t)n, d_tmp_dup, tb_dup, d_dig_sorted, d_rows_sorted, d_flags, d_nflag, ctx->stream));
@@ -392,11 +451,16 @@
                                 longest_label_run(lab_sorted, n) > kTilesLongestRun;
     if (ix_tiles && !tiles_hopeless) plan = mg::index_plan((uint32_t)n, E, s, sp->rs, t->s, maxv, dens0, ix_verify);
     else if (tiles_hopeless) plan.why = "a clade of more rows than a bucket's sort takes";
-    if (lb_made && !(plan.ok && memcmp(&plan.g, &early_plan.g, sizeof plan.g) == 0)) lb_made = false;
+    if (lb_made && !(plan.ok && memcmp(&plan.g, &early_plan.g, sizeof plan.g) == 0)) lb_made = cnt_made = false;
+    if (plan.ok && !lb_made) {
+        if (!ix_front) plan.front = false;
+        stat_zeroed = false;
+    }
+    if (lb_made) plan.front = early_plan.front;
     temp_bytes = std::max(std::max(mg::sparse_order_temp_bytes((uint32_t)n), mg::sparse_order_slice_temp_bytes((uint32_t)n)),
                           mg::sparse_offsets_temp_bytes((uint32_t)n));
     want_order = !ctx_opt(ctx, "MASHGPU_SPARSE_NO_ORDER");
-    ok = temp.alloc(std::max<size_t>(temp_bytes, 16)) == hipSuccess && gs_of.alloc(E) == hipSuccess && d_stat.alloc(1) == hipSuccess &&
+    ok = temp.alloc(std::max<size_t>(temp_bytes, 16)) == hipSuccess && gs_of.alloc(E) == hipSuccess && (d_stat.p != nullptr || d_stat.alloc(1) == hipSuccess) &&
               d_slots.alloc(std::max(mg::sparse_stat_scratch_bytes(), mg::index_stat_scratch_bytes())) == hipSuccess &&
               (!want_order || (key64_a.alloc(n) == hipSuccess && key64_b.alloc(n) == hipSuccess));
     ok = ok && take(&sp->off, n + 1) && take(&sp->keys_sorted, E) && take(&sp->gend, E) && take(&sp->sorted_rows, E) &&
@@ -473,14 +537,15 @@
 int SparseIndexBuild::build_by_tiles()
 {
     if (ok && e == hipSuccess && plan.ok) {
-        DevBuf<unsigned char> d_tcnt(ctx), d_start(ctx), d_big(ctx), d_pk(ctx), d_tc(ctx);
-        if ((lb_made || d_lb.alloc(plan.lb_bytes) == hipSuccess) && d_tcnt.alloc(plan.cnt_bytes) == hipSuccess && d_start.alloc(plan.start_bytes) == hipSuccess &&
+        DevBuf<unsigned char> d_start(ctx), d_big(ctx), d_pk(ctx), d_tc(ctx);
+        const uint64_t *Ht = H ? H : t->hashes;
+        if ((lb_made || d_lb.alloc(plan.lb_bytes) == hipSuccess) && (cnt_made || d_tcnt.alloc(plan.cnt_bytes) == hipSuccess) && d_start.alloc(plan.start_bytes) == hipSuccess &&
             d_big.alloc(plan.big_bytes) == hipSuccess && d_pk.alloc(plan.pk_bytes) == hipSuccess && d_tc.alloc(plan.tc_bytes) == hipSuccess) {
-            e = hipMemsetAsync(d_stat, 0, sizeof(Stat), ctx->stream);
+            e = stat_zeroed ? hipSuccess : hipMemsetAsync(d_stat, 0, sizeof(Stat), ctx->stream);
             if (e == hipSuccess)
-                e = mg::index_build(plan, H, sp->off, d_lb, d_tcnt, d_start, d_big, d_pk, d_tc, sp->keys_sorted, sp->sorted_rows, sp->gend, gs_of, sp->code_img,
+                e = mg::index_build(plan, Ht, sp->off, d_lb, d_tcnt, d_start, d_big, d_pk, d_tc, sp->keys_sorted, sp->sorted_rows, sp->gend, gs_of, sp->code_img,
                                     sp->pos_img, d_slots, &d_stat.p->shared, &d_stat.p->max_group, &d_stat.p->groups, d_stat.p->ixf, nullptr, ctx->stream,
-                                    lb_made ? 1 | 8 : 1);
+                                    lb_made ? (cnt_made ? 1 | 8 | 16 : 1 | 8) : 1, rowmap);
             DevBuf<uint32_t> d_swapped(ctx);
             if (e == hipSuccess && ctx_opt(ctx, "MASHGPU_IX_DEBUG_SWAP") && d_swapped.alloc(1) == hipSuccess) {
                 e = hipMemsetAsync(d_swapped, 0, 4, ctx->stream);
@@ -498,9 +563,9 @@
             }
             if (e == hipSuccess && ctx->aside_at_sort) ctx->aside_at_sort();
             if (e == hipSuccess)
-                e = mg::index_build(plan, H, sp->off, d_lb, d_tcnt, d_start, d_big, d_pk, d_tc, sp->keys_sorted, sp->sorted_rows, sp->gend, gs_of, sp->code_img,
+                e = mg::index_build(plan, Ht, sp->off, d_lb, d_tcnt, d_start, d_big, d_pk, d_tc, sp->keys_sorted, sp->sorted_rows, sp->gend, gs_of, sp->code_img,
                                     sp->pos_img, d_slots, &d_stat.p->shared, &d_stat.p->max_group, &d_stat.p->groups, d_stat.p->ixf,
-                                    lead_ready ? &lead : nullptr, ctx->stream, 2);
+                                    lead_ready ? &lead : nullptr, ctx->stream, 2, rowmap);
             if (e == hipSuccess && lead_ready) {
                 e = mg::dense_join_leaders(d_key, d_val, lead_cap, d_keyj, d_valj, d_cnt_sub, d_off_sub, d_nlead, ctx->stream);
                 if (e == hipSuccess) e = hipMemcpyAsync(lead_tot, d_nlead, 8, hipMemcpyDeviceToHost, ctx->stream);
@@ -510,9 +575,9 @@
             if (e == hipSuccess) e = hipEventCreateWithFlags(&ev_stats, hipEventDisableTiming);
             if (e == hipSuccess) e = hipEventRecord(ev_stats, ctx->stream);
             if (e == hipSuccess)
-                e = mg::index_build(plan, H, sp->off, d_lb, d_tcnt, d_start, d_big, d_pk, d_tc, sp->keys_sorted, sp->sorted_rows, sp->gend, gs_of, sp->code_img,
+                e = mg::index_build(plan, Ht, sp->off, d_lb, d_tcnt, d_start, d_big, d_pk, d_tc, sp->keys_sorted, sp->sorted_rows, sp->gend, gs_of, sp->code_img,
                                     sp->pos_img, d_slots, &d_stat.p->shared, &d_stat.p->max_group, &d_stat.p->groups, d_stat.p->ixf,
-                                    lead_ready ? &lead : nullptr, ctx->stream, 4);
+                                    lead_ready ? &lead : nullptr, ctx->stream, 4, rowmap);
             if (e == hipSuccess && want_order)
                 e = mg::launch_sparse_row_order(sp->off, sp->code_img, sp->gend, sp->rep, (uint32_t)n, sp->rs, temp, temp_bytes, key64_a, key64_b,
                                                 sp->order, ctx->stream);
@@ -540,9 +605,9 @@
                     if (e == hipSuccess) e = hipMemsetAsync(d_nlead, 0, 8, ctx->stream);
                     if (e == hipSuccess) e = hipMemsetAsync(d_stat.p, 0, offsetof(Stat, bad), ctx->stream);
                     if (e == hipSuccess)
-                        e = mg::index_build(plan, H, sp->off, d_lb, d_tcnt, d_start, d_big, d_pk, d_tc, sp->keys_sorted, sp->sorted_rows, sp->gend, gs_of,
+                        e = mg::index_build(plan, Ht, sp->off, d_lb, d_tcnt, d_start, d_big, d_pk, d_tc, sp->keys_sorted, sp->sorted_rows, sp->gend, gs_of,
                                             sp->code_img, sp->pos_img, d_slots, &d_stat.p->shared, &d_stat.p->max_group, &d_stat.p->groups, d_stat.p->ixf, &lead,
-                                            ctx->stream, 2);
+                                            ctx->stream, 2, rowmap);
                     if (e == hipSuccess) e = mg::dense_join_leaders(d_key, d_val, lead_cap, d_keyj, d_valj, d_cnt_sub, d_off_sub, d_nlead, ctx->stream);
                     if (e == hipSuccess) e = hipMemcpyAsync(lead_tot, d_nlead, 8, hipMemcpyDeviceToHost, ctx->stream);
                     if (e == hipSuccess) e = hipMemcpyAsync(&h_stat, d_stat, sizeof(Stat), hipMemcpyDeviceToHost, ctx->stream);
@@ -556,8 +621,8 @@
             }
             lead_done = built && lead_ready;
             if (ctx_opt(ctx, "MASHGPU_SPARSE_DBG"))
-                fprintf(stderr, "compare sparse: index by tiles: shift %u, %u buckets (%u per window, %u windows), fullest %u, %u beyond the LDS (%u values streamed)%s\n",
-                        plan.g.shift, plan.g.Bp, plan.g.BW, plan.g.NW, h_stat.ixf[mg::IXF_MAXBUCKET], h_stat.ixf[mg::IXF_NBIG], h_stat.ixf[mg::IXF_NSTREAMED],
+                fprintf(stderr, "compare sparse: index by tiles: %sshift %u, %u buckets (%u per window, %u windows), fullest %u, %u beyond the LDS (%u values streamed)%s%s\n",
+                        plan.front ? "fused front, " : "", plan.g.shift, plan.g.Bp, plan.g.BW, plan.g.NW, h_stat.ixf[mg::IXF_MAXBUCKET], h_stat.ixf[mg::IXF_NBIG], h_stat.ixf[mg::IXF_NSTREAMED], rowmap ? ", through the row map" : "",
                         h_stat.ixf[mg::IXF_DEGENERATE] ? " -- clumped values: sorted instead" : "");
         } else {
             (void)hipGetLastError();
@@ -578,6 +643,7 @@
 int SparseIndexBuild::build_by_sort()
 {
     if (ok && e == hipSuccess && (!built || ix_verify)) {
+        if ((e = need_copy(built ? "the sort beside the tiles (verify)" : "the general sort")) != hipSuccess) return MG_OK;
         const size_t sort_bytes = mg::sparse_sort_temp_bytes(E, end_bit, sort_begin_bit);
         DevBuf<unsigned char> temp_sort(ctx), d_ties(ctx);
         DevBuf<uint64_t> keys_a(ctx), v_keys(ctx);
diff --git a/mash_amd/csrc/index_build.h b/mash_amd/csrc/index_build.h
--- a/mash_amd/csrc/index_build.h
+++ b/mash_amd/csrc/index_build.h
@@ -30,17 +30,23 @@
     bool ok = false;
     const char *why = "";
     size_t lb_bytes = 0, cnt_bytes = 0, start_bytes = 0, big_bytes = 0, pk_bytes = 0, tc_bytes = 0;
+    bool front = false;
+    size_t front_lds_bytes = 0;
 };
 
 enum { IXF_NSTREAMED = 0, IXF_DEGENERATE = 1, IXF_MAXBUCKET = 2, IXF_NBIG = 3 };
 
-IxPlan index_plan(uint32_t n, uint32_t E, uint32_t s, uint32_t rs, uint64_t stride, uint64_t maxv, double dens0, bool want_gs);
+size_t index_front_lds_bytes();
+IxPlan index_plan(uint32_t n, uint32_t E, uint32_t s, uint32_t rs, uint64_t stride, uint64_t maxv, double dens0, bool want_gs,
+                  size_t front_lds = ~(size_t)0);
 size_t index_stat_scratch_bytes();
 hipError_t index_debug_swap(const IxPlan &plan, void *pk, const void *start, uint32_t *done, hipStream_t stream);
 hipError_t index_build(const IxPlan &plan, const uint64_t *hashes, const uint32_t *off, void *lb, void *cnt, void *start, void *big, void *pk, void *tc,
                        uint64_t *keys_sorted, uint32_t *sorted_rows, uint32_t *gend, uint32_t *gs_of, uint32_t *code_img, uint32_t *pos_img,
                        void *stat_scratch, unsigned long long *incidences, uint32_t *max_group, uint32_t *groups, uint32_t *flags,
-                       const IxLeaders *leaders, hipStream_t stream, int stages = 7);
+                       const IxLeaders *leaders, hipStream_t stream, int stages = 7, const uint32_t *rowmap = nullptr);
+hipError_t index_front(const IxPlan &plan, const uint64_t *hashes, const uint32_t *rowmap, const uint32_t *cnt_table, const uint32_t *off, void *lb,
+                       void *cnt, uint32_t *flags, hipStream_t stream);
 hipError_t index_gather_rows(const IxPlan &plan, const uint64_t *hashes, const uint32_t *inv, const uint32_t *cnt_table, uint64_t *out, void *lb,
                              hipStream_t stream);
 
diff --git a/mash_amd/csrc/index_build.hip b/mash_amd/csrc/index_build.hip
--- a/mash_amd/csrc/index_build.hip
+++ b/mash_amd/csrc/index_build.hip
@@ -136,12 +136,14 @@
     for (uint32_t x = (uint32_t)(wl + 1) + tid; x <= g.NW; x += 256u) o[x] = (uint16_t)cnt;
 }
 
-__global__ __launch_bounds__(256) void ix_window_offsets_kernel(IxGeom g, const uint64_t *H, const uint32_t *off, uint16_t *lb)
+__global__ __launch_bounds__(256) void ix_window_offsets_kernel(IxGeom g, const uint64_t *H, const uint32_t *rowmap, const uint32_t *cnt_table, const uint32_t *off,
+                                                                uint16_t *lb)
 {
     const uint32_t row = blockIdx.x * 4u + (threadIdx.x >> 6), lane = threadIdx.x & 63u;
     if (row < g.n) {
-        const uint32_t cnt = off[row + 1] - off[row];
-        const uint64_t *src = H + (uint64_t)row * g.stride;
+        const uint32_t tr = rowmap ? rowmap[row] : row;
+        const uint32_t cnt = cnt_table ? cnt_table[tr] : off[row + 1] - off[row];
+        const uint64_t *src = H + (uint64_t)tr * g.stride;
         uint16_t *out = lb + (uint64_t)row * (g.NW + 1u);
         const uint32_t wsh = g.shift + g.bw_log;
         for (uint32_t p = lane; p < cnt; p += 64u) {
@@ -154,10 +156,77 @@
     }
 }
 
+constexpr uint32_t IXF_NT = 1024;
+constexpr uint32_t IXF_UNR = 16;
+constexpr uint32_t IXF_LDS_BYTES = 152u * 1024u;
+static_assert(IX_RB / (IXF_NT / 64u) <= 64u, "a lane per row of the wave");
+
+__global__ __launch_bounds__(IXF_NT) void ix_front_kernel(IxGeom g, const uint64_t *__restrict__ H, const uint32_t *__restrict__ rowmap,
+                                                          const uint32_t *__restrict__ cnt_table, const uint32_t *__restrict__ off,
+                                                          uint16_t *__restrict__ lb, uint32_t *__restrict__ cnt, uint32_t *flags)
+{
+    MG_DYN_SHARED(uint32_t, s_h);
+    const uint32_t blk = blockIdx.x, tid = threadIdx.x, lane = tid & 63u, wave = tid >> 6, nwave = blockDim.x >> 6;
+    const uint32_t row0 = blk * IX_RB, nrows = g.n - row0 < IX_RB ? g.n - row0 : IX_RB;
+    for (uint32_t x = tid; x < (g.Bp + 1u) / 2u; x += blockDim.x) s_h[x] = 0;
+    uint32_t my_tr = 0, my_cnt = 0;
+    {
+        const uint32_t r = wave + lane * nwave;
+        if (r < nrows) {
+            my_tr = rowmap ? rowmap[row0 + r] : row0 + r;
+            my_cnt = cnt_table ? cnt_table[my_tr] : off[row0 + r + 1u] - off[row0 + r];
+        }
+    }
+    __syncthreads();
+    const uint32_t wsh = g.shift + g.bw_log;
+    int bad = 0;
+    for (uint32_t j = 0; wave + j * nwave < nrows; j++) {
+        const uint32_t a = row0 + wave + j * nwave;
+        const uint32_t tr = __shfl(my_tr, j), c = __shfl(my_cnt, j);
+        const uint64_t *src = H + (uint64_t)tr * g.stride;
+        uint16_t *o = lb + (uint64_t)a * (g.NW + 1u);
+        const uint64_t vlast = src[c > 0 ? c - 1u : 0u];
+        int wcarry = -1;
+        for (uint32_t base = 0; base < c; base += 64u * IXF_UNR) {
+            uint64_t v[IXF_UNR];
+#pragma unroll
+            for (uint32_t k = 0; k < IXF_UNR; k++) {
+                const uint32_t p = base + k * 64u + lane;
+                v[k] = src[p < c ? p : 0u];
+            }
+#pragma unroll
+            for (uint32_t k = 0; k < IXF_UNR; k++) {
+                const uint32_t p = base + k * 64u + lane;
+                const uint64_t b64 = v[k] >> g.shift;
+                const int w = b64 < (uint64_t)g.Bp ? (int)(uint32_t)(v[k] >> wsh) : (int)g.NW;
+                const int before = __shfl_up(w, 1u);
+                const int wp = lane > 0 ? before : wcarry;
+                wcarry = __shfl(w, 63u);
+                if (p < c) {
+                    if (b64 < (uint64_t)g.Bp) {
+                        const uint32_t b = (uint32_t)b64, h16 = (b & 1u) * 16u;
+                        const uint32_t old = atomicAdd(&s_h[b >> 1], 1u << h16);
+                        if (((old >> h16) & 0xFFFFu) == 0xFFFFu) bad = 1;
+                        for (int x = wp + 1; x <= w; x++) o[x] = (uint16_t)p;
+                    } else {
+                        bad = 1;
+                    }
+                }
+            }
+        }
+        const uint64_t bl = vlast >> g.shift;
+        const int wl = c > 0 ? (bl < (uint64_t)g.Bp ? (int)(uint32_t)(vlast >> wsh) : (int)g.NW) : -1;
+        for (uint32_t x = (uint32_t)(wl + 1) + lane; x <= g.NW; x += 64u) o[x] = (uint16_t)c;
+    }
+    bad = __syncthreads_or(bad);
+    for (uint32_t b = tid; b < g.Bp; b += blockDim.x) cnt[(uint64_t)blk * g.Bp + b] = (s_h[b >> 1] >> ((b & 1u) * 16u)) & 0xFFFFu;
+    if (bad && tid == 0) flags[IXF_DEGENERATE] = 1u;
+}
+
 constexpr uint32_t IX_ROUNDS = IX_RB / (IX_NT / IX_LPR);
 
-__global__ __launch_bounds__(IX_NT) void ix_tile_count_kernel(IxGeom g, const uint64_t *__restrict__ H, const uint16_t *__restrict__ lb,
-                                                              uint32_t *__restrict__ cnt)
+__global__ __launch_bounds__(IX_NT) void ix_tile_count_kernel(IxGeom g, const uint64_t *__restrict__ H, const uint32_t *__restrict__ rowmap,
+                                                              const uint16_t *__restrict__ lb, uint32_t *__restrict__ cnt)
 {
     __shared__ uint32_t s_hist[IX_BW_MAX];
     uint32_t blk = 0, w = 0;
@@ -165,29 +234,28 @@
     const uint32_t tid = threadIdx.x, sub = tid % IX_LPR;
     const uint32_t row0 = blk * IX_RB, nrows = g.n - row0 < IX_RB ? g.n - row0 : IX_RB;
     if (tid < g.BW) s_hist[tid] = 0;
-    uint32_t lo[IX_ROUNDS], hi[IX_ROUNDS];
+    uint32_t lo[IX_ROUNDS], hi[IX_ROUNDS], tr[IX_ROUNDS];
 #pragma unroll
     for (uint32_t it = 0; it < IX_ROUNDS; it++) {
-        const uint32_t r = it * (IX_NT / IX_LPR) + tid / IX_LPR;
-        const uint16_t *p = lb + (uint64_t)(row0 + (r < nrows ? r : 0u)) * (g.NW + 1u) + w;
+        const uint32_t r = it * (IX_NT / IX_LPR) + tid / IX_LPR, rc = row0 + (r < nrows ? r : 0u);
+        const uint16_t *p = lb + (uint64_t)rc * (g.NW + 1u) + w;
         const uint32_t a = p[0], b = p[1];
         lo[it] = a;
         hi[it] = r < nrows ? b : a;
+        tr[it] = rowmap ? rowmap[rc] : rc;
     }
     uint64_t v[IX_ROUNDS];
 #pragma unroll
     for (uint32_t it = 0; it < IX_ROUNDS; it++) {
-        const uint32_t r = it * (IX_NT / IX_LPR) + tid / IX_LPR;
         const bool in = lo[it] + sub < hi[it];
-        v[it] = H[in ? (uint64_t)(row0 + r) * g.stride + lo[it] + sub : (uint64_t)row0 * g.stride];
+        v[it] = H[in ? (uint64_t)tr[it] * g.stride + lo[it] + sub : (uint64_t)row0 * g.stride];
     }
     __syncthreads();
 #pragma unroll
     for (uint32_t it = 0; it < IX_ROUNDS; it++) {
-        const uint32_t r = it * (IX_NT / IX_LPR) + tid / IX_LPR;
         if (lo[it] + sub < hi[it]) {
             atomicAdd(&s_hist[(uint32_t)(v[it] >> g.shift) & (g.BW - 1u)], 1u);
-            const uint64_t *src = H + (uint64_t)(row0 + r) * g.stride;
+            const uint64_t *src = H + (uint64_t)tr[it] * g.stride;
             for (uint32_t k = lo[it] + sub + IX_LPR; k < hi[it]; k += IX_LPR) atomicAdd(&s_hist[(uint32_t)(src[k] >> g.shift) & (g.BW - 1u)], 1u);
         }
     }
@@ -219,13 +287,14 @@
 {
     __shared__ uint32_t s_part[16], s_max[16];
     const uint32_t tid = threadIdx.x;
+    const bool refused = flags[IXF_DEGENERATE] != 0u;
     uint32_t carry = 0, mx = 0;
     for (uint32_t base = 0; base < g.Bp; base += 4096u) {
         const uint32_t b = base + 4u * tid;
         uint32_t c[4], sum = 0;
 #pragma unroll
         for (uint32_t k = 0; k < 4u; k++) {
-            c[k] = b + k < g.Bp ? start[b + k] : 0u;
+            c[k] = b + k < g.Bp && !refused ? start[b + k] : 0u;
             sum += c[k];
             mx = c[k] > mx ? c[k] : mx;
             if (c[k] > IX_CAP) biglist[atomicAdd(&flags[IXF_NBIG], 1u)] = b + k;
@@ -301,8 +370,8 @@
                    IXL_ROWPRE = IXL_CNT + 16u * IX_NT * 2u, IXL_LO = IXL_ROWPRE + (IX_RB + 2u) * 4u, IXL_HIST = IXL_LO + IX_RB * 2u,
                    IXL_GBASE = IXL_HIST + (IX_BW_MAX + 2u) * 4u, IXL_PART = IXL_GBASE + IX_BW_MAX * 4u, IXL_BYTES = IXL_PART + 64u;
 
-__global__ __launch_bounds__(IX_NT, 4) void ix_tile_partition_kernel(IxGeom g, const uint64_t *__restrict__ H, const uint16_t *__restrict__ lb,
-                                                                  const uint32_t *__restrict__ colpre, const uint32_t *__restrict__ start,
+__global__ __launch_bounds__(IX_NT, 4) void ix_tile_partition_kernel(IxGeom g, const uint64_t *__restrict__ H, const uint32_t *__restrict__ rowmap,
+                                                                  const uint16_t *__restrict__ lb, const uint32_t *__restrict__ colpre, const uint32_t *__restrict__ start,
                                                                   const uint32_t *__restrict__ flags, uint64_t *__restrict__ pk,
                                                                   uint32_t *__restrict__ slot_img)
 {
@@ -317,9 +386,16 @@
     uint32_t *s_part = reinterpret_cast<uint32_t *>(lds + IXL_PART);
     uint32_t blk = 0, w = 0;
     if (!ix_tile_id(g, blk, w)) return;
+    const uint32_t refused = flags[IXF_DEGENERATE];
     const uint32_t tid = threadIdx.x, sub = tid % IX_LPR;
     IX_CLK_BEGIN();
     const uint32_t row0 = blk * IX_RB, nrows = g.n - row0 < IX_RB ? g.n - row0 : IX_RB;
+    uint32_t tr[IX_ROUNDS];
+#pragma unroll
+    for (uint32_t it = 0; it < IX_ROUNDS; it++) {
+        const uint32_t r = it * (IX_NT / IX_LPR) + tid / IX_LPR, rc = row0 + (r < nrows ? r : 0u);
+        tr[it] = rowmap ? rowmap[rc] : rc;
+    }
     uint32_t len = 0, gb = 0;
     if (tid < g.BW) {
         const uint32_t bg = w * g.BW + tid;
@@ -333,7 +409,7 @@
     }
     uint32_t total = 0;
     const uint32_t pre = ix_block_scan_sum(len, s_part, total);
-    if (total == 0) return;
+    if (total == 0 || refused != 0u) return;
     s_rowpre[tid] = pre;
     if (tid == IX_NT - 1u) s_rowpre[IX_NT] = total;
     if (tid < g.BW) {
@@ -354,7 +430,7 @@
             const uint32_t i = rp + sub;
             const bool in = sub < ln && i >= i0 && i < i0 + np;
             at[it] = in ? i - i0 : 0xFFFFFFFFu;
-            v[it] = H[in ? (uint64_t)(row0 + r) * g.stride + s_lo[rc] + sub : (uint64_t)row0 * g.stride];
+            v[it] = H[in ? (uint64_t)tr[it] * g.stride + s_lo[rc] + sub : (uint64_t)row0 * g.stride];
         }
 #pragma unroll
         for (uint32_t it = 0; it < IX_ROUNDS; it++) {
@@ -370,7 +446,7 @@
         for (uint32_t r = tid / IX_LPR; r < nrows; r += IX_NT / IX_LPR) {
             const uint32_t rp = s_rowpre[r], ln = s_rowpre[r + 1u] - rp;
             if (ln <= IX_LPR || rp + ln <= i0 || rp >= i0 + np) continue;
-            const uint64_t *src = H + (uint64_t)(row0 + r) * g.stride + s_lo[r];
+            const uint64_t *src = H + (uint64_t)(rowmap ? rowmap[row0 + r] : row0 + r) * g.stride + s_lo[r];
             for (uint32_t k = sub + IX_LPR; k < ln; k += IX_LPR) {
                 const uint32_t i = rp + k;
                 if (i < i0 || i >= i0 + np) continue;
@@ -448,6 +524,7 @@
     const uint32_t per = gridDim.x >> 3;
     const uint32_t q = (blockIdx.x & 7u) * per + (blockIdx.x >> 3);
     if (q >= g.nblk * nchunk) return;
+    if (flags[IXF_DEGENERATE] != 0u) return;
     const uint32_t blk = q / nchunk, ch = q - blk * nchunk;
     const uint32_t tid = threadIdx.x, quad = tid & 7u, rsub = tid >> 3;
     const uint32_t p0 = ch * IX5_CH + quad * 4u;
@@ -1106,7 +1183,9 @@
 }
 #endif
 
-IxPlan index_plan(uint32_t n, uint32_t E, uint32_t s, uint32_t rs, uint64_t stride, uint64_t maxv, double dens0, bool want_gs)
+size_t index_front_lds_bytes() { return IXF_LDS_BYTES; }
+
+IxPlan index_plan(uint32_t n, uint32_t E, uint32_t s, uint32_t rs, uint64_t stride, uint64_t maxv, double dens0, bool want_gs, size_t front_lds)
 {
     IxPlan p;
     IxGeom &g = p.g;
@@ -1149,8 +1228,26 @@
     p.tc_bytes = (size_t)E * 8u;
     p.big_bytes = ((size_t)E / IX_CAP + 2u) * 4u;
     if (p.lb_bytes > ((size_t)2 << 30) || p.cnt_bytes > ((size_t)2 << 30)) { p.why = "scratch of the tiles too large"; return p; }
+    p.front_lds_bytes = ((size_t)g.Bp + 1u) / 2u * 4u;
+    p.front = p.front_lds_bytes <= (front_lds < IXF_LDS_BYTES ? front_lds : (size_t)IXF_LDS_BYTES);
     p.ok = true;
     return p;
+}
+
+hipError_t index_front(const IxPlan &plan, const uint64_t *hashes, const uint32_t *rowmap, const uint32_t *cnt_table, const uint32_t *off, void *lb_v,
+                       void *cnt_v, uint32_t *flags, hipStream_t stream)
+{
+    if (!plan.ok || (cnt_table == nullptr && off == nullptr)) return hipErrorInvalidValue;
+    const IxGeom g = plan.g;
+    if (!plan.front) {
+        hipLaunchKernelGGL(ix_window_offsets_kernel, dim3((g.n + 3u) / 4u), dim3(256), 0, stream, g, hashes, rowmap, cnt_table, off, static_cast<uint16_t *>(lb_v));
+        return hipGetLastError();
+    }
+    const hipError_t e = hipFuncSetAttribute(reinterpret_cast<const void *>(ix_front_kernel), hipFuncAttributeMaxDynamicSharedMemorySize, (int)plan.front_lds_bytes);
+    if (e != hipSuccess) return e;
+    hipLaunchKernelGGL(ix_front_kernel, dim3(g.nblk), dim3(IXF_NT), plan.front_lds_bytes, stream, g, hashes, rowmap, cnt_table, off, static_cast<uint16_t *>(lb_v),
+                       static_cast<uint32_t *>(cnt_v), flags);
+    return hipGetLastError();
 }
 
 hipError_t index_gather_rows(const IxPlan &plan, const uint64_t *hashes, const uint32_t *inv, const uint32_t *cnt_table, uint64_t *out, void *lb_v,
@@ -1189,7 +1286,7 @@
 hipError_t index_build(const IxPlan &plan, const uint64_t *hashes, const uint32_t *off, void *lb_v, void *cnt_v, void *start_v, void *big_v, void *pk_v, void *tc_v,
                        uint64_t *keys_sorted, uint32_t *sorted_rows, uint32_t *gend, uint32_t *gs_of, uint32_t *code_img, uint32_t *pos_img,
                        void *stat_scratch, unsigned long long *incidences, uint32_t *max_group, uint32_t *groups, uint32_t *flags,
-                       const IxLeaders *leaders, hipStream_t stream, int stages)
+                       const IxLeaders *leaders, hipStream_t stream, int stages, const uint32_t *rowmap)
 {
     if (!plan.ok) return hipErrorInvalidValue;
     const IxGeom g = plan.g;
@@ -1202,13 +1299,18 @@
         e = hipFuncSetAttribute(reinterpret_cast<const void *>(ix_tile_partition_kernel), hipFuncAttributeMaxDynamicSharedMemorySize, (int)IXL_BYTES);
         if (e != hipSuccess) return e;
         const uint32_t tiles = 8u * ((g.nseq + 7u) / 8u);
-        if (!(stages & 8)) hipLaunchKernelGGL(ix_window_offsets_kernel, dim3((g.n + 3u) / 4u), dim3(256), 0, stream, g, hashes, off, lb);
-        hipLaunchKernelGGL(ix_tile_count_kernel, dim3(tiles), dim3(IX_NT), 0, stream, g, hashes, (const uint16_t *)lb, cnt);
+        bool cnt_made = (stages & 8) && (stages & 16);
+        if (!(stages & 8)) {
+            e = index_front(plan, hashes, rowmap, nullptr, off, lb_v, cnt_v, flags, stream);
+            if (e != hipSuccess) return e;
+            cnt_made = plan.front;
+        }
+        if (!cnt_made) hipLaunchKernelGGL(ix_tile_count_kernel, dim3(tiles), dim3(IX_NT), 0, stream, g, hashes, rowmap, (const uint16_t *)lb, cnt);
         hipLaunchKernelGGL(ix_col_scan_kernel, dim3((g.Bp + 255u) / 256u), dim3(256), 0, stream, g, cnt, start);
         hipLaunchKernelGGL(ix_bucket_scan_kernel, dim3(1), dim3(1024), 0, stream, g, start, flags, static_cast<uint32_t *>(big_v));
         e = hipGetLastError();
         if (e != hipSuccess) return e;
-        hipLaunchKernelGGL(ix_tile_partition_kernel, dim3(tiles), dim3(IX_NT), IXL_BYTES, stream, g, hashes, (const uint16_t *)lb, (const uint32_t *)cnt,
+        hipLaunchKernelGGL(ix_tile_partition_kernel, dim3(tiles), dim3(IX_NT), IXL_BYTES, stream, g, hashes, rowmap, (const uint16_t *)lb, (const uint32_t *)cnt,
                            (const uint32_t *)start, (const uint32_t *)flags, pk, pos_img);
         e = hipGetLastError();
         if (e != hipSuccess) return e;
```

Measured after the change: 443.6 billion pairs/s, median of 6. +2.0%, better.
